# LasseWolter/laughter-detection-icsi

Measured on AMD Instinct MI355X. Metric: 1 s@16 kHz segments/sec (featurize+ResNet fwd/bwd), higher is better.
Workload: dtype f32 (64->64 and 32->32 convolutions: f16x2 split operands with per-tile power-of-two scales, f32 accumulate; error vs float64 within 1.5x of the exact-f32 kernels'); 1 GPU; BASELINE configs[2]: end-to-end featurize (HIP fbank 44 mel) + ResNetBigger resnet_base fwd/bwd + clip + Adam, random labels, dropout 0.5; global_batch=512, parallelism=dp1, overlap_wgrad=False, overlap_wgrad_small=True, bf16x3_convs=True, f16x2_convs=True, relu_bits=True, virtual_a1=True

## Files before the change

include/lad_hip.h:

```cpp
#ifndef LAD_HIP_H
#define LAD_HIP_H

#include <stdint.h>

#ifdef __cplusplus
extern "C" {
#endif

#define LAD_VERSION 100

enum lad_status {
    LAD_OK = 0,
    LAD_ERR_INVALID = -1,
    LAD_ERR_HIP = -2,
    LAD_ERR_NOMEM = -3,
    LAD_NOT_COVERED = 1
};

int lad_version(void);
const char *lad_last_error(void);

enum lad_pad_mode {
    LAD_PAD_KALDI_MIRROR = 0,
    LAD_PAD_CENTER_REFLECT = 1,
// ... 53 lines not shown

int64_t lad_act_rows(int64_t batch, int32_t H, int32_t W);

int64_t lad_conv_packed_weight_floats(int32_t cout, int32_t cin, int32_t taps, int32_t mode);
int lad_conv_pack_weights(const float *w, int32_t cout, int32_t cin, int32_t taps, int32_t mode, float *wt,
                          void *stream);
int lad_conv_pack_weights_multi(const void *descs, int32_t n_desc, void *stream);
int64_t lad_conv_num_tiles(int64_t batch, int32_t H, int32_t W);
int lad_conv_fwd(const float *in, const float *wt, const float *bias, const float *addend, float *out,
                 float *stat_partials, int64_t batch, int32_t H, int32_t W, int32_t cin, int32_t cout, int32_t taps,
                 void *stream);
int lad_conv_s2_fwd(const float *in, const float *wt, const float *bias, float *out, float *stat_partials,
                    int64_t batch, int32_t H, int32_t W, int32_t cin, int32_t cout, int32_t taps, void *stream);
int lad_bn_fold(const float *gamma, const float *beta, const float *running_mean, const float *running_var,
                const float *conv_bias, int32_t channels, float *scale, float *shift, void *stream);
int lad_conv_fwd_eval(const float *in, const float *wt, const float *scale, const float *shift, const float *addend,
                      float *out, int64_t batch, int32_t H, int32_t W, int32_t cin, int32_t cout, int32_t taps,
                      int32_t relu, void *stream);
int lad_conv_s2_fwd_eval(const float *in, const float *wt, const float *scale, const float *shift, float *out,
                         int64_t batch, int32_t H, int32_t W, int32_t cin, int32_t cout, int32_t taps, int32_t relu,
                         void *stream);
int lad_upsample2(const float *src, float *up, int64_t batch, int32_t H, int32_t W, int32_t channels, void *stream);
int lad_conv_s2_dgrad(const float *dout, const float *wt, float *dx, int64_t batch, int32_t H, int32_t W, int32_t cin,
                      int32_t cout, int32_t taps, int32_t accumulate, void *stream);
int64_t lad_conv_s2_wgrad_workspace_floats(int32_t cin, int32_t cout, int32_t taps);
int lad_conv_s2_wgrad(const float *in, const float *dout, float *workspace, float *dw, float *dbias, int64_t batch, int32_t H,
                      int32_t W, int32_t cin, int32_t cout, int32_t taps, void *stream);
int64_t lad_conv_s2_wgrad_fused_workspace_floats(int32_t cin, int32_t cout);
int lad_conv_s2_wgrad_fused(const float *in, const float *dout, const float *dout_sc, float *workspace, float *dw,
                            float *dbias, float *dw_sc, int64_t batch, int32_t H, int32_t W, int32_t cin, int32_t cout,
                            void *stream);
int lad_conv_s2_fwd_fused(const float *in, const float *wt, const float *bias, const float *wt_sc, float *out,
                          float *stat_partials, float *out_sc, float *stat_partials_sc, int64_t batch, int32_t H, int32_t W,
                          int32_t cin, int32_t cout, void *stream);
int lad_conv_s2_dgrad_fused(const float *dout, const float *wt, const float *dout_sc, const float *wt_sc, float *dx,
                            int64_t batch, int32_t H, int32_t W, int32_t cin, int32_t cout, void *stream);
int64_t lad_conv_s2b3_packed_weight_bytes(void);
int lad_conv_s2b3_pack_weights(const float *w, const float *w_sc, void *wt, void *stream);
int lad_conv_s2b3_fwd(const float *in, const void *wt, const float *bias, float *out, float *stat_partials, float *out_sc,
                      float *stat_partials_sc, int64_t batch, int32_t H, int32_t W, void *stream);
int64_t lad_conv_s2b3_dgrad_packed_weight_bytes(void);
int lad_conv_s2b3_dgrad_pack_weights(const float *w, const float *w_sc, void *wt, void *stream);
int lad_conv_s2b3_pack_weights_pair(const float *w, const float *w_sc, void *wt_fwd, void *wt_dgrad, void *stream);
int64_t lad_conv_s2b3_dgrad_partials(int64_t batch, int32_t H, int32_t W);
int lad_conv_s2b3_dgrad(const float *dout, const float *dout_sc, const void *wt, float *dx, float *stat_partials, const float *bn_x,
                        const uint64_t *bn_bits, const float *bn_coef, int64_t batch, int32_t H, int32_t W, void *stream);
int64_t lad_conv_s2_dgrad_partials(int64_t batch, int32_t H, int32_t W);
int lad_conv_s2_dgrad_fused_bnstat(const float *dout, const float *wt, const float *dout_sc, const float *wt_sc, float *dx,
                                   float *stat_partials, const float *bn_x, const uint64_t *bn_bits, const float *bn_coef,
                                   int64_t batch, int32_t H, int32_t W, int32_t cin, int32_t cout, void *stream);
int64_t lad_conv_wgrad_workspace_floats(int32_t cin, int32_t cout, int32_t taps);
int lad_conv_wgrad(const float *in, const float *dout, float *workspace, float *dw, float *dbias, int64_t batch,
                   int32_t H, int32_t W, int32_t cin, int32_t cout, int32_t taps, void *stream);

int64_t lad_conv_b3_packed_weight_bytes(void);
int lad_conv_b3_pack_weights(const float *w, int32_t mode, void *wt, void *stream);
int lad_conv_b3_fwd_f32(const float *in, const void *wt, const float *bias, const float *addend, float *out,
                        float *partials, int64_t batch, int32_t H, int32_t W, void *stream);
int lad_conv_b3_fwd_f32_gated(const float *in, const void *wt, const float *bias, const float *addend,
                              const uint64_t *addend_bits, float *out, float *partials, int64_t batch, int32_t H,
                              int32_t W, void *stream);
int lad_conv_b3_dgrad_bnstat(const float *in, const void *wt, const float *addend, const uint64_t *addend_bits,
                             float *out, float *stat_partials, const float *bn_x, const uint64_t *bn_bits,
                             const float *bn_coef, int64_t batch, int32_t H, int32_t W, void *stream);
int64_t lad_conv_b3c_packed_weight_bytes(int32_t channels);
int lad_conv_b3c_pack_weights(const float *w, int32_t mode, void *wt, int32_t channels, void *stream);
int lad_conv_b3c_fwd_f32(const float *in, const void *wt, const float *bias, const float *addend, float *out,
                         float *partials, int64_t batch, int32_t H, int32_t W, int32_t channels, void *stream);
int lad_conv_b3c_dgrad_bnstat(const float *in, const void *wt, const float *addend, float *out, float *stat_partials,
                              const float *bn_x, const float *bn_coef, int64_t batch, int32_t H, int32_t W,
                              int32_t channels, void *stream);
int lad_conv_b3c_fwd_f32_bnrelu(const float *in, const float *in_coef, const void *wt, const float *bias, float *out,
                                float *partials, int64_t batch, int32_t H, int32_t W, int32_t channels, void *stream);
int64_t lad_conv_h2_packed_weight_bytes(int32_t channels);
int lad_conv_h2_pack_weights_multi(const void *table, int32_t n, int32_t channels, void *stream);
int lad_conv_wgrad_h2(const float *in, const float *in_coef, const float *dout, float *workspace, float *dw, float *dbias,
                      int64_t batch, int32_t H, int32_t W, int32_t channels, void *stream);
int lad_conv_wgrad_h2_bnbwd(const float *in, const float *in_coef, const float *dy, const float *bn_x, const uint64_t *bn_bits,
                            const float *bn_coef, const float *bcoef, float *dc, float *workspace, float *dw, float *dbias,
                            int64_t batch, int32_t H, int32_t W, int32_t channels, void *stream);
int lad_conv_h2(const float *in, const float *in_coef, const void *wt, const float *bias, const float *addend,
                const uint64_t *addend_bits, float *out, float *partials, const float *bn_x, const uint64_t *bn_bits,
                const float *bn_coef, int64_t batch, int32_t H, int32_t W, int32_t channels, void *stream);
int64_t lad_conv_wgrad_b3c_workspace_floats(int32_t channels);
int lad_conv_wgrad_b3c(const float *in, const float *in_coef, const float *dout, float *workspace, float *dw, float *dbias,
                       int64_t batch, int32_t H, int32_t W, int32_t channels, void *stream);
int lad_conv_b3_fwd_f32_bnrelu(const float *in, const float *in_coef, const void *wt, const float *bias, float *out,
                               float *partials, int64_t batch, int32_t H, int32_t W, void *stream);
int lad_conv_wgrad_b3_bnrelu(const float *in, const float *in_coef, const float *dout, float *workspace, float *dw,
                             float *dbias, int64_t batch, int32_t H, int32_t W, void *stream);
int lad_wgrad_defer_begin(void);
int lad_wgrad_defer_flush(void *stream);
int lad_conv_wgrad_b3(const float *in, const float *dout, float *workspace, float *dw, float *dbias, int64_t batch,
                      int32_t H, int32_t W, void *stream);

int lad_stem_fwd(const float *feat, const float *weight, float *out, float *stat_partials, int64_t batch, int32_t H,
                 int32_t W, int32_t cout, void *stream);
int lad_stem_fwd_eval(const float *feat, const float *weight, const float *scale, const float *shift, float *out,
                      int64_t batch, int32_t H, int32_t W, int32_t cout, int64_t frame_stride, int64_t frames_avail,
                      void *stream);
int64_t lad_stem_moments_workspace_doubles(void);
int64_t lad_stem_moments_doubles(void);
int lad_stem_bn_stats(const float *feat, const float *weight, const float *gamma, const float *beta, float *running_mean,
                      float *running_var, float momentum, float *coef, double *moments, double *workspace, int64_t batch, int32_t H,
                      int32_t W, int32_t cout, void *stream);
int64_t lad_stem_bwd_onepass_workspace_floats(void);
int lad_stem_bwd_onepass(const float *feat, const float *weight, const float *dy, const float *coef, const float *gamma,
                         const double *moments, float *workspace, float *dw, float *dgamma, float *dbeta, int64_t batch, int32_t H,
                         int32_t W, int32_t cout, void *stream);
int64_t lad_stem_wgrad_workspace_floats(void);
int lad_stem_wgrad(const float *feat, const float *dout, float *workspace, float *dw, int64_t batch, int32_t H,
                   int32_t W, int32_t cout, void *stream);
int lad_stem_wgrad_bn(const float *feat, const float *dy, const float *x, const float *weight, const float *coef,
                      const float *bcoef, float *workspace, float *dw, int64_t batch, int32_t H, int32_t W, int32_t cout,
                      void *stream);
int64_t lad_stem_bn_bwd_groups(int64_t batch, int32_t H, int32_t W);
int lad_stem_bn_bwd_sums(const float *feat, const float *weight, const float *dy, const float *coef, float *partials,
                         int64_t batch, int32_t H, int32_t W, int32_t cout, void *stream);

int lad_bn_finalize(float *stat_partials, int64_t n_tiles, int32_t channels, int64_t count, const float *gamma,
                    const float *beta, float *running_mean, float *running_var, float momentum, float *coef,
                    void *stream);
int lad_bn_finalize_pair(float *stat_partials_a, float *stat_partials_b, int64_t n_tiles, int32_t channels, int64_t count,
                         const float *gamma_a, const float *beta_a, float *running_mean_a, float *running_var_a, float *coef_a,
                         const float *gamma_b, const float *beta_b, float *running_mean_b, float *running_var_b, float *coef_b,
                         float momentum, void *stream);
int lad_bn_act(const float *x, const float *coef, const float *res, const float *res_coef, float *y, int64_t batch,
               int32_t H, int32_t W, int32_t channels, int32_t relu, void *stream);
int64_t lad_bn_bwd_workspace_floats(int32_t channels);
int lad_bn_bwd(const float *dy, const float *y, const float *x, const float *coef, const float *gamma,
               const float *xs, const float *scoef, const float *sgamma, float *dx, float *aux, float *dgamma,
               float *dbeta, float *dsgamma, float *dsbeta, float *workspace, float *bcoef, float *pre_partials,
               int64_t pre_tiles, int64_t batch, int32_t H, int32_t W, int32_t channels, int32_t relu, int32_t mode,
               void *stream);
int lad_bn_act_bits(const float *x, const float *coef, const float *res, const float *res_coef, float *y,
                    uint64_t *y_bits, int64_t batch, int32_t H, int32_t W, int32_t channels, void *stream);
int lad_bn_bwd_bits(const float *dy, const uint64_t *y_bits, const float *x, const float *coef, const float *gamma,
                    float *dx, float *dgamma, float *dbeta, float *workspace, float *bcoef, float *pre_partials,
                    int64_t pre_tiles, int64_t batch, int32_t H, int32_t W, int32_t channels, void *stream);
int lad_conv_fwd_bnstat(const float *in, const float *wt, const float *addend, float *out, float *stat_partials,
                        const float *bn_x, const float *bn_y, const float *bn_coef, int64_t batch, int32_t H, int32_t W,
                        int32_t cin, int32_t cout, int32_t taps, void *stream);

int lad_pool_fwd(const float *x, float *pooled, int64_t batch, int32_t H, int32_t W, int32_t channels, void *stream);
int lad_pool_bwd(const float *dpooled, float *dx, int64_t batch, int32_t H, int32_t W, int32_t channels, void *stream);
int64_t lad_head_workspace_floats(int64_t batch, int32_t F);
int lad_head_fwd_train(const float *const *params, const float *pooled, int64_t batch, int32_t F, const float *drop1,
                       const float *drop2, const int32_t *labels, float momentum, float *h, float *stats,
                       float *probs, float *metrics, void *stream);
int lad_head_fwd_train_rng(const float *const *params, const float *pooled, int64_t batch, int32_t F, float *drop1, float *drop2, float keep,
                           uint64_t seed, int64_t *rng_counter, int64_t *nbt, int32_t n_nbt, const int32_t *labels, float momentum,
                           float *h, float *stats, float *probs, float *metrics, void *stream);
int lad_head_fwd_eval(const float *const *params, const float *pooled, int64_t batch, int32_t F, float *probs,
                      void *stream);
int lad_bce_metrics(const float *probs, const int32_t *labels, int64_t n, float *metrics, void *stream);
int lad_head_bwd(const float *const *params, float *const *grads, const float *pooled, const float *h,
                 const float *stats, const float *probs, const float *dprobs, int64_t batch, int32_t F,
                 const float *drop1, const float *drop2, const int32_t *labels, float *workspace, float *dpooled,
                 void *stream);

int64_t lad_f16_packed_weight_halfs(int32_t cout, int32_t cin, int32_t taps);
int lad_f16_pack_weights(const float *w, int32_t cout, int32_t cin, int32_t taps, void *wt, void *stream);
int lad_f16_stem_fwd(const float *feat, const float *weight, const float *scale, const float *shift, void *out,
                     int64_t batch, int32_t H, int32_t W, int32_t cout, int64_t frame_stride, int64_t frames_avail,
                     void *stream);
int lad_f16_conv_fwd(const void *in, const void *wt, const float *scale, const float *shift, const void *addend, void *out,
// ... 162 lines not shown
```

laughter-detection-icsi_amd/_hip.py:

```python
import ctypes
import os

import numpy as np
import torch

_HERE = os.path.dirname(os.path.abspath(__file__))
LIB_PATH = os.environ.get("LAD_HIP_LIB") or os.path.join(_HERE, "liblad_hip.so")

c_void_p = ctypes.c_void_p
c_int = ctypes.c_int
c_i64 = ctypes.c_int64
c_float = ctypes.c_float
c_double = ctypes.c_double
c_i32 = ctypes.c_int32
c_float_p = ctypes.POINTER(ctypes.c_float)


class LadHipError(RuntimeError):
    pass


class FbankCfg(ctypes.Structure):
    _fields_ = [("n_fft", ctypes.c_int32), ("frame_len", ctypes.c_int32), ("hop", ctypes.c_int32),
                ("n_mels", ctypes.c_int32), ("n_mfcc", ctypes.c_int32), ("pad_mode", ctypes.c_int32),
                ("log_mode", ctypes.c_int32), ("remove_dc", ctypes.c_int32), ("preemph", ctypes.c_float),
                ("log_floor", ctypes.c_float)]


class AugmentParams(ctypes.Structure):
    _fields_ = [("seed", ctypes.c_uint64), ("epoch", ctypes.c_uint32), ("p", ctypes.c_float), ("mix_p", ctypes.c_float),
                ("snr_lo", ctypes.c_float), ("snr_hi", ctypes.c_float), ("gain_lo", ctypes.c_float), ("gain_hi", ctypes.c_float),
                ("W", ctypes.c_int32), ("n_time", ctypes.c_int32), ("Wt", ctypes.c_int32), ("n_freq", ctypes.c_int32),
                ("Wf", ctypes.c_int32)]


SIGNATURES = {
    "lad_version": (c_int, []),
    "lad_last_error": (ctypes.c_char_p, []),
    "lad_fbank_plan_create": (c_int, [ctypes.POINTER(FbankCfg), c_void_p, c_void_p, c_void_p,
                                      ctypes.POINTER(c_void_p)]),
    "lad_fbank_plan_destroy": (c_int, [c_void_p]),
    "lad_fbank_plan_set_kernel": (c_int, [c_void_p, c_int]),
    "lad_fbank_plan_has_fast_kernel": (c_int, [c_void_p]),
    "lad_fbank_num_frames": (c_i64, [c_void_p, c_i64]),
    "lad_fbank_forward": (c_int, [c_void_p, c_void_p, c_i64, c_i64, c_void_p, c_void_p]),
    "lad_fbank_forward_long": (c_int, [c_void_p, c_void_p, c_i64, c_void_p, c_void_p]),
    "lad_gather_segments": (c_int, [c_void_p] * 5 + [c_i64, c_i32, c_i32, c_float, c_void_p, c_void_p]),
    "lad_gather_segments_aug": (c_int, [c_void_p] * 5 + [c_i64, c_i32, c_i32, c_float, ctypes.POINTER(AugmentParams), c_void_p, c_i32, c_i64,
                                        c_void_p, c_void_p]),
    "lad_assemble_windows": (c_int, [c_void_p, c_void_p, c_void_p, c_i64, c_i32, c_i32, c_i32, c_i32, c_void_p]),
    "lad_act_rows": (c_i64, [c_i64, c_i32, c_i32]),
    "lad_conv_packed_weight_floats": (c_i64, [c_i32, c_i32, c_i32, c_i32]),
    "lad_conv_pack_weights": (c_int, [c_void_p, c_i32, c_i32, c_i32, c_i32, c_void_p, c_void_p]),
    "lad_conv_pack_weights_multi": (c_int, [c_void_p, c_i32, c_void_p]),
    "lad_conv_num_tiles": (c_i64, [c_i64, c_i32, c_i32]),
    "lad_conv_fwd": (c_int, [c_void_p] * 6 + [c_i64, c_i32, c_i32, c_i32, c_i32, c_i32, c_void_p]),
    "lad_conv_b3_packed_weight_bytes": (c_i64, []),
    "lad_conv_b3_pack_weights": (c_int, [c_void_p, c_i32, c_void_p, c_void_p]),
    "lad_conv_b3_fwd_f32": (c_int, [c_void_p] * 6 + [c_i64, c_i32, c_i32, c_void_p]),
    "lad_conv_b3c_packed_weight_bytes": (c_i64, [c_i32]),
    "lad_conv_b3c_pack_weights": (c_int, [c_void_p, c_i32, c_void_p, c_i32, c_void_p]),
    "lad_conv_b3c_fwd_f32": (c_int, [c_void_p] * 6 + [c_i64, c_i32, c_i32, c_i32, c_void_p]),
    "lad_conv_b3c_fwd_f32_bnrelu": (c_int, [c_void_p] * 6 + [c_i64, c_i32, c_i32, c_i32, c_void_p]),
    "lad_conv_b3c_dgrad_bnstat": (c_int, [c_void_p] * 7 + [c_i64, c_i32, c_i32, c_i32, c_void_p]),
    "lad_conv_h2_packed_weight_bytes": (c_i64, [c_i32]),
    "lad_conv_h2_pack_weights_multi": (c_int, [c_void_p, c_i32, c_i32, c_void_p]),
    "lad_conv_wgrad_h2": (c_int, [c_void_p] * 6 + [c_i64, c_i32, c_i32, c_i32, c_void_p]),
    "lad_conv_h2": (c_int, [c_void_p] * 11 + [c_i64, c_i32, c_i32, c_i32, c_void_p]),
    "lad_conv_wgrad_h2_bnbwd": (c_int, [c_void_p] * 11 + [c_i64, c_i32, c_i32, c_i32, c_void_p]),
    "lad_conv_wgrad_b3c_workspace_floats": (c_i64, [c_i32]),
    "lad_conv_wgrad_b3c": (c_int, [c_void_p] * 6 + [c_i64, c_i32, c_i32, c_i32, c_void_p]),
    "lad_conv_b3_fwd_f32_gated": (c_int, [c_void_p] * 7 + [c_i64, c_i32, c_i32, c_void_p]),
    "lad_conv_b3_fwd_f32_bnrelu": (c_int, [c_void_p] * 6 + [c_i64, c_i32, c_i32, c_void_p]),
    "lad_conv_wgrad_b3_bnrelu": (c_int, [c_void_p] * 6 + [c_i64, c_i32, c_i32, c_void_p]),
    "lad_wgrad_defer_begin": (c_int, []),
    "lad_wgrad_defer_flush": (c_int, [c_void_p]),
    "lad_conv_b3_dgrad_bnstat": (c_int, [c_void_p] * 9 + [c_i64, c_i32, c_i32, c_void_p]),
    "lad_conv_wgrad_b3": (c_int, [c_void_p] * 5 + [c_i64, c_i32, c_i32, c_void_p]),
    "lad_conv_s2_fwd": (c_int, [c_void_p] * 5 + [c_i64, c_i32, c_i32, c_i32, c_i32, c_i32, c_void_p]),
    "lad_bn_fold": (c_int, [c_void_p] * 5 + [c_i32, c_void_p, c_void_p, c_void_p]),
    "lad_conv_fwd_eval": (c_int, [c_void_p] * 6 + [c_i64, c_i32, c_i32, c_i32, c_i32, c_i32, c_i32, c_void_p]),
    "lad_conv_s2_fwd_eval": (c_int, [c_void_p] * 5 + [c_i64, c_i32, c_i32, c_i32, c_i32, c_i32, c_i32, c_void_p]),
    "lad_upsample2": (c_int, [c_void_p, c_void_p, c_i64, c_i32, c_i32, c_i32, c_void_p]),
    "lad_conv_s2_dgrad": (c_int, [c_void_p] * 3 + [c_i64, c_i32, c_i32, c_i32, c_i32, c_i32, c_i32, c_void_p]),
    "lad_conv_s2_wgrad_workspace_floats": (c_i64, [c_i32, c_i32, c_i32]),
    "lad_conv_s2_fwd_fused": (c_int, [c_void_p] * 8 + [c_i64, c_i32, c_i32, c_i32, c_i32, c_void_p]),
    "lad_conv_s2_dgrad_partials": (c_i64, [c_i64, c_i32, c_i32]),
    "lad_conv_s2b3_packed_weight_bytes": (c_i64, []),
    "lad_conv_s2b3_pack_weights": (c_int, [c_void_p, c_void_p, c_void_p, c_void_p]),
    "lad_conv_s2b3_fwd": (c_int, [c_void_p] * 7 + [c_i64, c_i32, c_i32, c_void_p]),
    "lad_conv_s2b3_dgrad_packed_weight_bytes": (c_i64, []),
    "lad_conv_s2b3_dgrad_pack_weights": (c_int, [c_void_p, c_void_p, c_void_p, c_void_p]),
    "lad_conv_s2b3_pack_weights_pair": (c_int, [c_void_p] * 5),
    "lad_conv_s2b3_dgrad_partials": (c_i64, [c_i64, c_i32, c_i32]),
    "lad_conv_s2b3_dgrad": (c_int, [c_void_p] * 8 + [c_i64, c_i32, c_i32, c_void_p]),
    "lad_conv_s2_dgrad_fused_bnstat": (c_int, [c_void_p] * 9 + [c_i64, c_i32, c_i32, c_i32, c_i32, c_void_p]),
    "lad_conv_s2_dgrad_fused": (c_int, [c_void_p] * 5 + [c_i64, c_i32, c_i32, c_i32, c_i32, c_void_p]),
    "lad_conv_s2_wgrad_fused_workspace_floats": (c_i64, [c_i32, c_i32]),
    "lad_conv_s2_wgrad_fused": (c_int, [c_void_p] * 7 + [c_i64, c_i32, c_i32, c_i32, c_i32, c_void_p]),
    "lad_conv_s2_wgrad": (c_int, [c_void_p] * 5 + [c_i64, c_i32, c_i32, c_i32, c_i32, c_i32, c_void_p]),
    "lad_conv_wgrad_workspace_floats": (c_i64, [c_i32, c_i32, c_i32]),
    "lad_conv_wgrad": (c_int, [c_void_p] * 5 + [c_i64, c_i32, c_i32, c_i32, c_i32, c_i32, c_void_p]),
    "lad_stem_fwd": (c_int, [c_void_p] * 4 + [c_i64, c_i32, c_i32, c_i32, c_void_p]),
    "lad_stem_fwd_eval": (c_int, [c_void_p] * 5 + [c_i64, c_i32, c_i32, c_i32, c_i64, c_i64, c_void_p]),
    "lad_stem_wgrad_workspace_floats": (c_i64, []),
    "lad_stem_wgrad": (c_int, [c_void_p] * 4 + [c_i64, c_i32, c_i32, c_i32, c_void_p]),
    "lad_stem_wgrad_bn": (c_int, [c_void_p] * 8 + [c_i64, c_i32, c_i32, c_i32, c_void_p]),
    "lad_stem_bn_bwd_groups": (c_i64, [c_i64, c_i32, c_i32]),
    "lad_stem_bn_bwd_sums": (c_int, [c_void_p] * 5 + [c_i64, c_i32, c_i32, c_i32, c_void_p]),
    "lad_bn_finalize": (c_int, [c_void_p, c_i64, c_i32, c_i64, c_void_p, c_void_p, c_void_p, c_void_p, c_float,
                                c_void_p, c_void_p]),
    "lad_stem_moments_workspace_doubles": (c_i64, []),
    "lad_stem_moments_doubles": (c_i64, []),
    "lad_stem_bn_stats": (c_int, [c_void_p] * 6 + [c_float] + [c_void_p] * 3 + [c_i64, c_i32, c_i32, c_i32, c_void_p]),
    "lad_stem_bwd_onepass_workspace_floats": (c_i64, []),
    "lad_stem_bwd_onepass": (c_int, [c_void_p] * 10 + [c_i64, c_i32, c_i32, c_i32, c_void_p]),
    "lad_bn_finalize_pair": (c_int, [c_void_p, c_void_p, c_i64, c_i32, c_i64] + [c_void_p] * 10 + [c_float, c_void_p]),
    "lad_bn_act": (c_int, [c_void_p] * 5 + [c_i64, c_i32, c_i32, c_i32, c_i32, c_void_p]),
    "lad_bn_bwd_workspace_floats": (c_i64, [c_i32]),
    "lad_bn_act_bits": (c_int, [c_void_p] * 6 + [c_i64, c_i32, c_i32, c_i32, c_void_p]),
    "lad_bn_bwd_bits": (c_int, [c_void_p] * 11 + [c_i64, c_i64, c_i32, c_i32, c_i32, c_void_p]),
    "lad_bn_bwd": (c_int, [c_void_p] * 17 + [c_i64, c_i64, c_i32, c_i32, c_i32, c_i32, c_i32, c_void_p]),
    "lad_conv_fwd_bnstat": (c_int, [c_void_p] * 8 + [c_i64, c_i32, c_i32, c_i32, c_i32, c_i32, c_void_p]),
    "lad_pool_fwd": (c_int, [c_void_p, c_void_p, c_i64, c_i32, c_i32, c_i32, c_void_p]),
    "lad_pool_bwd": (c_int, [c_void_p, c_void_p, c_i64, c_i32, c_i32, c_i32, c_void_p]),
    "lad_head_workspace_floats": (c_i64, [c_i64, c_i32]),
    "lad_head_fwd_train": (c_int, [c_void_p, c_void_p, c_i64, c_i32, c_void_p, c_void_p, c_void_p, c_float,
                                   c_void_p, c_void_p, c_void_p, c_void_p, c_void_p]),
    "lad_head_fwd_train_rng": (c_int, [c_void_p, c_void_p, c_i64, c_i32, c_void_p, c_void_p, c_float, ctypes.c_uint64, c_void_p, c_void_p, c_i32,
                                       c_void_p, c_float, c_void_p, c_void_p, c_void_p, c_void_p, c_void_p]),
    "lad_head_fwd_eval": (c_int, [c_void_p, c_void_p, c_i64, c_i32, c_void_p, c_void_p]),
    "lad_bce_metrics": (c_int, [c_void_p, c_void_p, c_i64, c_void_p, c_void_p]),
    "lad_head_bwd": (c_int, [c_void_p] * 7 + [c_i64, c_i32] + [c_void_p] * 6),
    "lad_f16_packed_weight_halfs": (c_i64, [c_i32, c_i32, c_i32]),
    "lad_f16_pack_weights": (c_int, [c_void_p, c_i32, c_i32, c_i32, c_void_p, c_void_p]),
    "lad_f16_stem_fwd": (c_int, [c_void_p] * 5 + [c_i64, c_i32, c_i32, c_i32, c_i64, c_i64, c_void_p]),
    "lad_f16_conv_fwd": (c_int, [c_void_p] * 6 + [c_i64, c_i32, c_i32, c_i32, c_i32, c_i32, c_i32, c_void_p]),
    "lad_f16_block_fwd": (c_int, [c_void_p] * 8 + [c_i64, c_i32, c_i32, c_i32, c_void_p]),
    "lad_f16_conv_s2_fwd_sc": (c_int, [c_void_p] * 9 + [c_i64, c_i32, c_i32, c_i32, c_i32, c_i32, c_void_p]),
    "lad_f16_conv_s2_fwd_mapped_sc": (c_int, [c_void_p] * 9 + [c_i64, c_i32, c_i32, c_i32, c_i32, c_i64, c_i64, c_i32, c_i64, c_i64, c_i32,
                                              c_i32, c_i32, c_i32, c_void_p]),
    "lad_f16_conv_s2_fwd": (c_int, [c_void_p] * 5 + [c_i64, c_i32, c_i32, c_i32, c_i32, c_i32, c_i32, c_void_p]),
    "lad_f16_conv_s2_fwd_windows": (c_int, [c_void_p] * 5 + [c_i64, c_i32, c_i32, c_i32, c_i32, c_i32, c_i32, c_i32, c_void_p]),
    "lad_f16_conv_s2_fwd_mapped": (c_int, [c_void_p] * 5 + [c_i64, c_i32, c_i32, c_i32, c_i32, c_i64, c_i64, c_i32, c_i64, c_i64, c_i32,
                                                          c_i32, c_i32, c_i32, c_i32, c_void_p]),
    "lad_f16_block_fwd_stem_rows": (c_int, [c_void_p, c_i64, c_i64, c_void_p, c_i64] + [c_void_p] * 10 + [c_i64, c_i32, c_i32, c_void_p]),
    "lad_f16_conv_s2_strips_fwd": (c_int, [c_void_p] * 9 + [c_i64, c_i32, c_i32, c_i32, c_i32, c_i64, c_i64, c_i64, c_i32, c_void_p]),
    "lad_f16_tail_fwd": (c_int, [c_void_p, c_i64, c_i32, c_i32, c_i32, c_i32, c_i64, c_i64, c_i32, c_i64, c_i64, c_void_p, c_void_p, c_i32,
                                 c_void_p, c_void_p]),
    "lad_f16_pool_fwd": (c_int, [c_void_p, c_void_p, c_i64, c_i32, c_i32, c_i32, c_void_p]),
    "lad_grad_sumsq_partials": (c_i32, []),
# ... 157 lines not shown
```

laughter-detection-icsi_amd/csrc/conv_h2.hip:

```cpp
#include "lad_common.h"
#include "lad_device.h"
#include "lad_b3_tile.h"
#include "lad_bn_math.h"
#include "lad_h2.h"

#include <algorithm>
#include <cstdlib>

namespace {
using namespace lad;
using namespace lad::b3t;

constexpr int KC = 32;
constexpr int ROWB = 128;
constexpr int FPIECES = KC * 4 / 16;

template <int C>
struct H2 {
    static constexpr int NSTAGE = C / KC;
    static constexpr int NCT = C / 16;
    static constexpr int PLANE_B = NCT * 1024;
    static constexpr int TAP_BYTES = 2 * PLANE_B;
    static constexpr int IMG_BYTES = TAPS * NSTAGE * TAP_BYTES;
    static constexpr int TAIL_BYTES = 16;
};

struct PackRec {
    const float *w;
    unsigned char *wt;
    int mode;
    int channels;
};
constexpr int PACK_SPLIT = 16;
template <int C>
__device__ __forceinline__ void pack_h2_image(const PackRec &rec, int part) {
    using K = H2<C>;
    __shared__ float smax[K::NSTAGE][16];
    __shared__ int kexp[K::NSTAGE];
    const int tid = threadIdx.x, lane = tid & 63, wave = tid >> 6;
    float m[K::NSTAGE];
#pragma unroll
    for (int s = 0; s < K::NSTAGE; ++s) m[s] = 0.f;
    static_assert((C * TAPS) % 4 == 0, "float4 groups stay inside one (co, ci range)");
    for (int idx4 = tid; idx4 < C * C * TAPS / 4; idx4 += 1024) {
        const float4 v = reinterpret_cast<const float4 *>(rec.w)[idx4];
        const float a[4] = {fabsf(v.x), fabsf(v.y), fabsf(v.z), fabsf(v.w)};
#pragma unroll
        for (int j = 0; j < 4; ++j) {
            const int idx = idx4 * 4 + j;
            const int co = idx / (C * TAPS), ci = (idx / TAPS) % C;
            const int k = rec.mode == 0 ? ci : co;
#pragma unroll
            for (int s = 0; s < K::NSTAGE; ++s) m[s] = (k / KC == s) ? fmaxf(m[s], a[j]) : m[s];
        }
    }
#pragma unroll
    for (int s = 0; s < K::NSTAGE; ++s) {
        const float v = wave_max64_dpp(m[s]);
        if (lane == 0) smax[s][wave] = v;
    }
    __syncthreads();
    if (tid < K::NSTAGE) {
        float v = 0.f;
        for (int w = 0; w < 16; ++w) v = fmaxf(v, smax[tid][w]);
        kexp[tid] = scale_exp(v);
        if (part == 0) reinterpret_cast<int *>(rec.wt + K::IMG_BYTES)[tid] = kexp[tid];
    }
    __syncthreads();
    unsigned short *out = reinterpret_cast<unsigned short *>(rec.wt);
    constexpr int SHARE = K::IMG_BYTES / 2 / PACK_SPLIT;
    for (int idx = part * SHARE + tid; idx < (part + 1) * SHARE; idx += 1024) {
        int t = idx;
        const int e = t & 7; t >>= 3;
        const int n = t & 15; t >>= 4;
        const int kq = t & 3; t >>= 2;
        const int ct = t % K::NCT; t /= K::NCT;
        const int plane = t & 1; t >>= 1;
        const int stage = t % K::NSTAGE;
        const int tap = t / K::NSTAGE;
        const int k = stage * KC + kq * 8 + e;
        const int nn = ct * 16 + n;
        const int co = rec.mode == 0 ? nn : k, ci = rec.mode == 0 ? k : nn;
        const int src_tap = rec.mode == 0 ? tap : TAPS - 1 - tap;
        const float v = rec.w[((int64_t)co * C + ci) * TAPS + src_tap] * pow2f(kexp[stage]);
        const _Float16 h1 = (_Float16)v;
        const _Float16 h2 = (_Float16)(v - (float)h1);
        out[idx] = __builtin_bit_cast(unsigned short, plane == 0 ? h1 : h2);
    }
}
template <int C>
__global__ __launch_bounds__(1024) void pack_h2_kernel(const PackRec *__restrict__ recs) {
    const PackRec rec = recs[blockIdx.x / PACK_SPLIT];
    const int part = blockIdx.x % PACK_SPLIT;
    if (C == 64 || (C == 0 && rec.channels == 64)) pack_h2_image<64>(rec, part);
    else pack_h2_image<32>(rec, part);
}

#ifdef LAD_STAMP
__device__ unsigned long long lad_dbg_h2[16 * 16384];
#define LAD_H2_STAMP(k) \
    if (threadIdx.x == 0 && blockIdx.x < 16384) lad_dbg_h2[blockIdx.x * 16 + (k)] = __builtin_amdgcn_s_memtime();
#else
#define LAD_H2_STAMP(k)
#endif

constexpr int NSLOT = 3;
constexpr int H2_EPI_ANY = -1;
constexpr int h2_epi(bool bias, int addend, bool partials, bool from_bits) {
    return (bias ? 1 : 0) | (addend << 1) | (partials ? 8 : 0) | (from_bits ? 16 : 0);
}
template <int C, int RB, bool STAT, bool INBN, int EPI>
__global__ __launch_bounds__(THREADS, RB == 1 ? 3 : 2) void conv_h2_kernel(const float *__restrict__ in, const unsigned char *__restrict__ wt,
                                                             const float *__restrict__ bias, const float *addend,
                                                             const unsigned long long *__restrict__ abits, float *out,
                                                             float *__restrict__ partials, Geom g, B3Stat bst,
                                                             const float *__restrict__ in_coef) {
    using K = H2<C>;
    constexpr int NSTAGE = K::NSTAGE, NCT = K::NCT, PLANE_B = K::PLANE_B, TAP_BYTES = K::TAP_BYTES;
    constexpr int TMW = TM * RB, NRT = 2 * RB;
    constexpr int NPRE = ((TMW + 2 * 47) * FPIECES + THREADS - 1) / THREADS;
    constexpr int CPS = TAPS;
    constexpr int KP = (CPS - NSLOT) < CPS / 2 ? (CPS - NSLOT) : CPS / 2;
    static_assert(CPS % NSLOT == 0 && NPRE <= 32, "every stage starts in ring slot 0; staging geometry");
    extern __shared__ __attribute__((aligned(128))) unsigned char smem_b[];
    const int tid = threadIdx.x, lane = tid & 63, wave = __builtin_amdgcn_readfirstlane(tid >> 6);
    const int halo = g.Wp + 1;
    const int nrows = TMW + 2 * halo;
    const int main_bytes = max(NSLOT * TAP_BYTES + nrows * ROWB, TM * (C + 4) * 4);
    unsigned char *b_s = smem_b;
    unsigned char *a_s = b_s + NSLOT * TAP_BYTES;
    unsigned char *mask_s = smem_b + main_bytes;
    float *smax = reinterpret_cast<float *>(mask_s + TMW);
    const unsigned per_x = (gridDim.x + 7u) / 8u;
    const unsigned tile_id = (blockIdx.x % 8u) * per_x + blockIdx.x / 8u;
    const int64_t q0 = (int64_t)tile_id * TMW;
    if (q0 >= g.rows) return;

    LAD_H2_STAMP(0)
    constexpr int NW_TAP = TAP_BYTES / (THREADS * 16);
    static_assert(TAP_BYTES % (THREADS * 16) == 0 && NW_TAP >= 1, "the DMA count per tap must not depend on the wave");
    auto issue_tap = [&](int tap, int stage, int slot) {
        const unsigned char *src = wt + (int64_t)(tap * NSTAGE + stage) * TAP_BYTES;
        unsigned char *dst = b_s + slot * TAP_BYTES;
#pragma unroll
        for (int r = 0; r < NW_TAP; ++r)
            dma16(src + (r * THREADS + tid) * 16, lds_addr(dst + (r * THREADS + wave * 64) * 16));
    };
    const int *wexp = reinterpret_cast<const int *>(wt + K::IMG_BYTES);

    const int64_t start = q0 - halo;
    const int64_t first = start < 0 ? 0 : start;
    const int row_lo = (int)(first - start);
    const int64_t span_rows = min(g.rows - first, (int64_t)(nrows - row_lo));
    auto voff = [&](int u) {
        const int idx = u * THREADS + tid;
        return idx < nrows * FPIECES ? ((idx >> 3) - row_lo) * (C * 4) + (idx & 7) * 16 : -1;
    };
    auto stage_rsrc = [&](int stage) {
        return make_rsrc(reinterpret_cast<const unsigned char *>(in) + first * (C * 4) + stage * (KC * 4), span_rows * (C * 4) - stage * (KC * 4));
    };
    unsigned keep_bits = 0;
    u32x4 pre[NPRE];
    auto activate = [&](int stage) {
        float m = 0.f;
        f32x4 sc = {0.f, 0.f, 0.f, 0.f}, sh = sc;
        if (INBN) {
            sc = *reinterpret_cast<const f32x4 *>(in_coef + stage * KC + (tid & 7) * 4);
            sh = *reinterpret_cast<const f32x4 *>(in_coef + C + stage * KC + (tid & 7) * 4);
        }
#pragma unroll
        for (int u = 0; u < NPRE; ++u) {
            if (INBN) pre[u] = bn_relu_piece(pre[u], sc, sh, (keep_bits >> u) & 1u);
            const float4 f = as_f4(pre[u]);
            m = fmaxf(fmaxf(m, fmaxf(fabsf(f.x), fabsf(f.y))), fmaxf(fabsf(f.z), fabsf(f.w)));
        }
        m = wave_max64_dpp(m);
        if (lane == 0) smax[wave] = m;
    };
    auto tile_exp = [&]() { return scale_exp(fmaxf(fmaxf(smax[0], smax[1]), fmaxf(smax[2], smax[3]))); };
    auto put_all = [&](float scl) {
#pragma unroll
        for (int u = 0; u < NPRE; ++u) {
            const int idx = u * THREADS + tid;
            if (idx < nrows * FPIECES) {
                const int row = idx >> 3, piece = idx & 7;
                const float4 f = as_f4(pre[u]);
                unsigned a1, a2, b1, b2;
                split2_pair(f.x * scl, f.y * scl, a1, a2);
                split2_pair(f.z * scl, f.w * scl, b1, b2);
                const unsigned off = (unsigned)row * ROWB + ((((piece >> 1) ^ (row & 6)) << 4) | ((piece & 1) << 3));
                *reinterpret_cast<u32x2 *>(a_s + off) = u32x2{a1, b1};
                *reinterpret_cast<u32x2 *>(a_s + (off ^ 64u)) = u32x2{a2, b2};
            }
        }
    };

    {
        const __amdgpu_buffer_rsrc_t in_r = stage_rsrc(0);
#pragma unroll
        for (int u = 0; u < NPRE; ++u) pre[u] = buf_load16(in_r, voff(u));
    }
#pragma unroll
    for (int k = 0; k < NSLOT - 1; ++k) issue_tap(k, 0, k);
    for (int j = tid; j < TMW; j += THREADS) mask_s[j] = interior_row32((uint32_t)q0 + (uint32_t)j, g) ? 1 : 0;
    if (INBN) {
#pragma unroll
        for (int u = 0; u < NPRE; ++u)
            keep_bits |= (interior_row32((uint32_t)(start + ((u * THREADS + tid) >> 3)), g) ? 1u : 0u) << u;
    }
    LAD_H2_STAMP(1)
    activate(0);
    __syncthreads();
    int ktot = tile_exp() + wexp[0];
    put_all(pow2f(ktot - wexp[0]));
    LAD_H2_STAMP(2)

    const int m = lane & 15, kq = lane >> 4;
    const int rl = wave * 32 + m + halo - 1;
    const unsigned char *b_lane = b_s + kq * 256 + m * 16;

    f32x4 acc[NRT][NCT];
#pragma unroll
    for (int r = 0; r < NRT; ++r)
#pragma unroll
        for (int c = 0; c < NCT; ++c) acc[r][c] = f32x4{0.f, 0.f, 0.f, 0.f};

#pragma unroll
    for (int stage = 0; stage < NSTAGE; ++stage) {
        const bool last = stage + 1 == NSTAGE;
#pragma unroll
        for (int tap = 0; tap < TAPS; ++tap) {
            const int kc = tap;
            const int slot = kc % NSLOT;
            {
                constexpr int YOUNGER = NSLOT - 2;
                if (!last) {
                    if (kc > KP && kc <= KP + NSLOT - 1) wait_dma_fixed<YOUNGER, NPRE, NW_TAP>();
                    else wait_dma_fixed<YOUNGER, 0, NW_TAP>();
                } else {
                    if (CPS - 1 - kc >= YOUNGER) wait_dma_fixed<YOUNGER, 0, NW_TAP>();
                    else wait_dma_fixed<0, 0, NW_TAP>();
                }
                __syncthreads();
                const int kn = kc + NSLOT - 1;
                if (kn < CPS) issue_tap(kn, stage, kn % NSLOT);
                else if (!last) issue_tap(kn - CPS, stage + 1, kn % NSLOT);
                if (kc == KP && !last) {
                    const __amdgpu_buffer_rsrc_t in_r = stage_rsrc(stage + 1);
#pragma unroll
                    for (int u = 0; u < NPRE; ++u) pre[u] = buf_load16(in_r, voff(u));
                }
            }
            const int rt = rl + (tap / 3 - 1) * g.Wp + (tap % 3);
            const unsigned a1o = (unsigned)rt * ROWB + ((unsigned)(kq ^ (rt & 6)) << 4);
            const unsigned a2o = a1o ^ 64u;
            const int boff = slot * TAP_BYTES;
            f16x8 a1[NRT], a2[NRT];
#pragma unroll
            for (int r = 0; r < NRT; ++r) {
                const int roff = ((r >> 1) * TM + (r & 1) * 16) * ROWB;
                a1[r] = *reinterpret_cast<const f16x8 *>(a_s + a1o + roff);
                a2[r] = *reinterpret_cast<const f16x8 *>(a_s + a2o + roff);
            }
#pragma unroll
            for (int c = 0; c < NCT; ++c) {
                const f16x8 b1 = *reinterpret_cast<const f16x8 *>(b_lane + boff + c * 1024);
                const f16x8 b2 = *reinterpret_cast<const f16x8 *>(b_lane + boff + PLANE_B + c * 1024);
#pragma unroll
                for (int r = 0; r < NRT; ++r) acc[r][c] = __builtin_amdgcn_mfma_f32_16x16x32_f16(a1[r], b2, acc[r][c], 0, 0, 0);
#pragma unroll
                for (int r = 0; r < NRT; ++r) acc[r][c] = __builtin_amdgcn_mfma_f32_16x16x32_f16(a2[r], b1, acc[r][c], 0, 0, 0);
#pragma unroll
                for (int r = 0; r < NRT; ++r) acc[r][c] = __builtin_amdgcn_mfma_f32_16x16x32_f16(a1[r], b1, acc[r][c], 0, 0, 0);
            }
        }
#ifdef LAD_STAMP
        if (threadIdx.x == 0 && blockIdx.x < 16384) lad_dbg_h2[blockIdx.x * 16 + 3 + 2 * stage] = __builtin_amdgcn_s_memtime();
#endif
        if (!last) {
            activate(stage + 1);
            __syncthreads();
            const int kw = wexp[stage + 1];
            const int kn = min(tile_exp() + kw, ktot + 8);
            const int d = kn - ktot;
            if (d != 0) {
#pragma unroll
                for (int r = 0; r < NRT; ++r)
#pragma unroll
                    for (int c = 0; c < NCT; ++c)
#pragma unroll
                        for (int j = 0; j < 4; ++j) acc[r][c][j] = __builtin_ldexpf(acc[r][c][j], d);
            }
            ktot = kn;
            const int ka = kn - kw;
            put_all(ka >= -126 ? pow2f(ka) : 0.f);
        }
#ifdef LAD_STAMP
        if (threadIdx.x == 0 && blockIdx.x < 16384) lad_dbg_h2[blockIdx.x * 16 + 4 + 2 * stage] = __builtin_amdgcn_s_memtime();
#endif
    }
    __syncthreads();
    LAD_H2_STAMP(11)
#pragma unroll
    for (int rb = 0; rb < RB; ++rb) {
        const int64_t qs = q0 + rb * TM;
        if (rb > 0) {
            if (qs >= g.rows) break;
            __syncthreads();
        }
        auto store_acc = [&](float *my) {
#pragma unroll
            for (int rr = 0; rr < 2; ++rr)
#pragma unroll
                for (int c = 0; c < NCT; ++c)
#pragma unroll
                    for (int j = 0; j < 4; ++j)
                        my[(rr * 16 + (lane >> 4) * 4 + j) * (C + 4) + c * 16 + m] = __builtin_ldexpf(acc[rb * 2 + rr][c][j], -ktot);
        };
        if constexpr (EPI == H2_EPI_ANY)
            b3_epilogue<C, STAT>(store_acc, bias, addend, abits, out, partials, mask_s + rb * TM, reinterpret_cast<float *>(smem_b), qs, g.rows, bst);
        else
            h2_epilogue<C, STAT, (EPI & 1) != 0, (EPI >> 1) & 3, (EPI & 8) != 0, (EPI & 16) != 0>(
                store_acc, bias, addend, abits, out, partials, mask_s + rb * TM, reinterpret_cast<float *>(smem_b), qs, g.rows, bst);
    }
    LAD_H2_STAMP(12)
}

template <int C, int RB>
size_t h2_lds_bytes(const Geom &g) {
    using K = H2<C>;
    const int nrows = TM * RB + 2 * (g.Wp + 1);
    const size_t main_bytes = std::max<size_t>(NSLOT * K::TAP_BYTES + (size_t)nrows * ROWB, (size_t)TM * (C + 4) * 4);
    return main_bytes + TM * RB + 16;
}

int h2_two_rounds() {
    static int n = 0;
    if (n == 0) {
        int dev = 0;
        hipDeviceProp_t prop;
        n = (hipGetDevice(&dev) == hipSuccess && hipGetDeviceProperties(&prop, dev) == hipSuccess && prop.multiProcessorCount > 0)
                ? 4 * prop.multiProcessorCount : 1024;
    }
    return n;
}

struct H2Args {
    const float *in, *in_coef;
    const unsigned char *wt;
    const float *bias, *addend;
    const unsigned long long *abits;
    float *out, *partials;
    B3Stat bst;
    Geom g;
    hipStream_t stream;
};

template <int C, int RB, bool STAT, bool INBN, int EPI>
int launch_h2_form(const H2Args &a) {
    static lad::DeviceOnce attr_set;
    if (!attr_set) {
        LAD_HIP_CHECK(hipFuncSetAttribute((const void *)conv_h2_kernel<C, RB, STAT, INBN, EPI>, hipFuncAttributeMaxDynamicSharedMemorySize, 96 * 1024));
        attr_set = true;
    }
    const int64_t tiles = ceil_div(a.g.rows, TM * RB);
    hipLaunchKernelGGL((conv_h2_kernel<C, RB, STAT, INBN, EPI>), dim3((unsigned)(ceil_div(tiles, 8) * 8)), dim3(THREADS), (h2_lds_bytes<C, RB>(a.g)),
                       a.stream, a.in, a.wt, a.bias, a.addend, a.abits, a.out, a.partials, a.g, a.bst, a.in_coef);
    return check_launch("conv_h2_kernel");
}

template <int C, int RB, bool STAT, bool INBN>
int launch_h2_rb(const H2Args &a) {
    const int form = h2_epi(a.bias != nullptr, a.addend == nullptr ? H2_ADD_NONE : a.abits == nullptr ? H2_ADD_PLAIN : H2_ADD_GATED,
                            a.partials != nullptr, STAT && a.bst.bits != nullptr);
#define LAD_H2_FORM(...)                                                                                                           \
    if (form == h2_epi(__VA_ARGS__)) return launch_h2_form<C, RB, STAT, INBN, h2_epi(__VA_ARGS__)>(a);
    if constexpr (STAT) {
        LAD_H2_FORM(false, H2_ADD_NONE, true, false)
        LAD_H2_FORM(false, H2_ADD_GATED, true, true)
    } else {
        LAD_H2_FORM(true, H2_ADD_NONE, true, false)
        LAD_H2_FORM(true, H2_ADD_PLAIN, true, false)
        if constexpr (!INBN) {
            LAD_H2_FORM(false, H2_ADD_NONE, false, false)
            LAD_H2_FORM(false, H2_ADD_PLAIN, false, false)
            LAD_H2_FORM(false, H2_ADD_GATED, false, false)
        }
    }
#undef LAD_H2_FORM
    return launch_h2_form<C, RB, STAT, INBN, H2_EPI_ANY>(a);
}

template <int C, bool STAT, bool INBN>
int launch_h2(const float *in, const float *in_coef, const void *wt, const float *bias, const float *addend, const uint64_t *abits,
              float *out, float *partials, const B3Stat &bst, int64_t batch, int32_t H, int32_t W, void *stream, const char *who) {
    const Geom g = make_geom(batch, H, W);
    LAD_REQUIRE(g.rows < ((int64_t)1 << 31) && g.img < (1 << 20), "%s: more than 2^31 rows, or an image of more than 2^20 positions", who);
    LAD_REQUIRE(W <= 46, "%s: image too wide for the tile (W = %d)", who, W);
    const H2Args a{in, in_coef, (const unsigned char *)wt, bias, addend, (const unsigned long long *)abits, out, partials, bst, g, (hipStream_t)stream};
    if (ceil_div(g.rows, TM * 2) < h2_two_rounds()) return launch_h2_rb<C, 1, STAT, INBN>(a);
    return launch_h2_rb<C, 2, STAT, INBN>(a);
}
}

extern "C" int64_t lad_conv_h2_packed_weight_bytes(int32_t channels) {
    if (channels == 64) return H2<64>::IMG_BYTES + H2<64>::TAIL_BYTES;
    if (channels == 32) return H2<32>::IMG_BYTES + H2<32>::TAIL_BYTES;
    return -1;
}

extern "C" int lad_conv_h2_pack_weights_multi(const void *table, int32_t n, int32_t channels, void *stream) {
    using namespace lad;
    LAD_REQUIRE(table && n >= 1, "lad_conv_h2_pack_weights_multi: empty table");
    static_assert(sizeof(PackRec) == 24, "record layout");
    if (channels == 64) hipLaunchKernelGGL(pack_h2_kernel<64>, dim3(n * PACK_SPLIT), dim3(1024), 0, (hipStream_t)stream, (const PackRec *)table);
    else if (channels == 32) hipLaunchKernelGGL(pack_h2_kernel<32>, dim3(n * PACK_SPLIT), dim3(1024), 0, (hipStream_t)stream, (const PackRec *)table);
    else if (channels == 0) hipLaunchKernelGGL(pack_h2_kernel<0>, dim3(n * PACK_SPLIT), dim3(1024), 0, (hipStream_t)stream, (const PackRec *)table);
    else return fail(LAD_ERR_INVALID, "lad_conv_h2_pack_weights_multi: 64 or 32 channels, or 0 = per record (got %d)", channels);
    return check_launch("pack_h2_kernel");
}

extern "C" int lad_conv_h2(const float *in, const float *in_coef, const void *wt, const float *bias, const float *addend,
                           const uint64_t *addend_bits, float *out, float *partials, const float *bn_x, const uint64_t *bn_bits,
                           const float *bn_coef, int64_t batch, int32_t H, int32_t W, int32_t channels, void *stream) {
    using namespace lad;
    const char *who = "lad_conv_h2";
    LAD_REQUIRE(batch >= 1 && H >= 1 && W >= 1, "%s: bad geometry", who);
    LAD_REQUIRE(in && wt && out, "%s: null buffer", who);
    LAD_REQUIRE(addend_bits == nullptr || addend != nullptr, "%s: sign bits without an addend", who);
    LAD_REQUIRE((const void *)in != (const void *)out, "%s: the convolution cannot run in place", who);
    const bool stat = bn_x != nullptr;
    LAD_REQUIRE(!stat || (partials && bn_coef), "%s: the BatchNorm sums need partials and bn_coef", who);
    LAD_REQUIRE(stat || bn_bits == nullptr, "%s: bn_bits without bn_x", who);
    LAD_REQUIRE(!(stat && in_coef), "%s: an input BatchNorm and the backward sums are not combined", who);
    LAD_REQUIRE(channels == 64 || (addend_bits == nullptr && bn_bits == nullptr), "%s: sign bits are kept for 64-channel activations only", who);
    const B3Stat bst{bn_x, (const unsigned long long *)bn_bits, bn_coef};
    if (channels == 64) {
        if (stat) return launch_h2<64, true, false>(in, nullptr, wt, bias, addend, addend_bits, out, partials, bst, batch, H, W, stream, who);
        if (in_coef) return launch_h2<64, false, true>(in, in_coef, wt, bias, addend, addend_bits, out, partials, bst, batch, H, W, stream, who);
        return launch_h2<64, false, false>(in, nullptr, wt, bias, addend, addend_bits, out, partials, bst, batch, H, W, stream, who);
    }
    if (channels == 32) {
        if (stat) return launch_h2<32, true, false>(in, nullptr, wt, bias, addend, addend_bits, out, partials, bst, batch, H, W, stream, who);
        if (in_coef) return launch_h2<32, false, true>(in, in_coef, wt, bias, addend, addend_bits, out, partials, bst, batch, H, W, stream, who);
        return launch_h2<32, false, false>(in, nullptr, wt, bias, addend, addend_bits, out, partials, bst, batch, H, W, stream, who);
    }
    return fail(LAD_ERR_INVALID, "%s: 64 or 32 channels (got %d)", who, channels);
}

#ifdef LAD_STAMP
extern "C" int lad_debug_read_h2_stamps(unsigned long long *host_dst, int64_t n) {
    return hipMemcpyFromSymbol(host_dst, HIP_SYMBOL(lad_dbg_h2), n * sizeof(unsigned long long)) == hipSuccess ? 0 : -2;
}
#endif
```

laughter-detection-icsi_amd/csrc/lad_b3_tile.h:

```cpp
#pragma once
#include "lad_common.h"
#include "lad_device.h"

namespace lad {
namespace b3t {

constexpr int TAPS = 9;
constexpr int TM = 128;
constexpr int THREADS = 256;

struct B3Stat {
    const float *x;
    const unsigned long long *bits;
    const float *coef;
};

struct B3Scatter {
    const int *rowoff;
    int64_t base_row;
    int64_t span_rows;
    int64_t part_tile;
};

template <int C, bool STAT, bool SCATTER = false, class StoreAcc, class MaskT>
__device__ __forceinline__ void b3_epilogue(StoreAcc store_acc, const float *__restrict__ bias, const float *addend,
                                            const unsigned long long *__restrict__ abits, float *out, float *__restrict__ partials,
                                            const MaskT *mask_tile, float *out_s, int64_t q0, int64_t rows, const B3Stat &bst,
                                            const B3Scatter &sct = B3Scatter{nullptr, 0, 0, 0}) {
    constexpr int LDO = C + 4, LPR = C / 4, RPI = 64 / LPR, ITER = 32 / RPI, STEP = RPI * C * 4;
    const int tid = (int)threadIdx.x, lane = tid & 63, wave = tid >> 6;
    float *my = out_s + wave * 32 * LDO;
    store_acc(my);
    const int c4 = lane % LPR, rsub = lane / LPR;
    const int64_t row0 = SCATTER ? sct.base_row : q0;
    const int64_t tile_rows = SCATTER ? sct.span_rows : rows - q0;
    const int64_t tile_bytes = tile_rows * (C * 4);
    const int voff = ((wave * 32 + rsub) * C + c4 * 4) * 4;
    const int woff = (wave * 32 + rsub) * 8;
    int ro[SCATTER ? ITER : 1];
    if (SCATTER) {
#pragma unroll
        for (int it = 0; it < ITER; ++it) ro[it] = sct.rowoff[wave * 32 + it * RPI + rsub];
    }
    auto off16 = [&](int it) { return SCATTER ? (ro[SCATTER ? it : 0] < 0 ? -1 : ro[SCATTER ? it : 0] * (C * 4) + c4 * 16) : voff + it * STEP; };
    auto off8 = [&](int it) { return SCATTER ? (ro[SCATTER ? it : 0] < 0 ? -1 : ro[SCATTER ? it : 0] * 8) : woff + it * RPI * 8; };
    const __amdgpu_buffer_rsrc_t out_r = make_rsrc(out + row0 * C, tile_bytes);
    f32x4 bv = {0.f, 0.f, 0.f, 0.f};
    if (bias != nullptr) bv = *reinterpret_cast<const f32x4 *>(bias + c4 * 4);
    f32x4 s1 = {0.f, 0.f, 0.f, 0.f}, s2 = s1;
    f32x4 fsc = s1, fsh = s1, mu = s1, is = s1, mul = s1, isl = s1;
    if (STAT) {
        fsc = *reinterpret_cast<const f32x4 *>(bst.coef + 0 * C + c4 * 4);
        fsh = *reinterpret_cast<const f32x4 *>(bst.coef + 1 * C + c4 * 4);
        mu = *reinterpret_cast<const f32x4 *>(bst.coef + 2 * C + c4 * 4);
        is = *reinterpret_cast<const f32x4 *>(bst.coef + 3 * C + c4 * 4);
        mul = *reinterpret_cast<const f32x4 *>(bst.coef + 4 * C + c4 * 4);
        isl = *reinterpret_cast<const f32x4 *>(bst.coef + 5 * C + c4 * 4);
    }
    const bool from_bits = STAT && bst.bits != nullptr;
    auto gate = [&](u32x4 v, u32x2 w) {
        const unsigned lo = w.x >> c4, hi = w.y >> c4;
        v.x = (lo & 1u) ? v.x : 0u;
        v.y = (lo & 0x10000u) ? v.y : 0u;
        v.z = (hi & 1u) ? v.z : 0u;
        v.w = (hi & 0x10000u) ? v.w : 0u;
        return v;
    };
    constexpr int NI = STAT ? ITER / 2 : ITER;
#pragma unroll
    for (int i0 = 0; i0 < ITER; i0 += NI) {
        u32x4 adv[NI], bx[STAT ? NI : 1];
        u32x2 wv[NI], bw[STAT ? NI : 1];
        if (addend != nullptr) {
            const __amdgpu_buffer_rsrc_t add_r = make_rsrc(addend + row0 * C, tile_bytes);
#pragma unroll
            for (int u = 0; u < NI; ++u) adv[u] = buf_load16(add_r, off16(i0 + u));
            if (abits != nullptr) {
                const __amdgpu_buffer_rsrc_t bits_r = make_rsrc(abits + row0, tile_rows * 8);
#pragma unroll
                for (int u = 0; u < NI; ++u) wv[u] = buf_load8(bits_r, off8(i0 + u));
            }
        }
        if (STAT) {
            const __amdgpu_buffer_rsrc_t x_r = make_rsrc(bst.x + row0 * C, tile_bytes);
#pragma unroll
// ... 86 lines not shown
        const unsigned lo = w.x >> c4, hi = w.y >> c4;
        v.x = (lo & 1u) ? v.x : 0u;
        v.y = (lo & 0x10000u) ? v.y : 0u;
        v.z = (hi & 1u) ? v.z : 0u;
        v.w = (hi & 0x10000u) ? v.w : 0u;
        return v;
    };
    constexpr int NI = (STAT || ADDEND == H2_ADD_GATED) ? ITER / 2 : ITER;
#pragma unroll
    for (int i0 = 0; i0 < ITER; i0 += NI) {
        u32x4 adv[ADDEND != H2_ADD_NONE ? NI : 1], bx[STAT ? NI : 1];
        u32x2 wv[ADDEND == H2_ADD_GATED ? NI : 1], bw[FROM_BITS ? NI : 1];
        if constexpr (ADDEND != H2_ADD_NONE) {
            const __amdgpu_buffer_rsrc_t add_r = make_rsrc(addend + q0 * C, tile_bytes);
#pragma unroll
            for (int u = 0; u < NI; ++u) adv[u] = buf_load16(add_r, voff + (i0 + u) * STEP);
            if constexpr (ADDEND == H2_ADD_GATED) {
                const __amdgpu_buffer_rsrc_t bits_r = make_rsrc(abits + q0, tile_rows * 8);
#pragma unroll
                for (int u = 0; u < NI; ++u) wv[u] = buf_load8(bits_r, woff + (i0 + u) * RPI * 8);
            }
        }
        if constexpr (STAT) {
            const __amdgpu_buffer_rsrc_t x_r = make_rsrc(bst.x + q0 * C, tile_bytes);
#pragma unroll
            for (int u = 0; u < NI; ++u) bx[u] = buf_load16(x_r, voff + (i0 + u) * STEP);
            if constexpr (FROM_BITS) {
                const __amdgpu_buffer_rsrc_t w_r = make_rsrc(bst.bits + q0, tile_rows * 8);
#pragma unroll
                for (int u = 0; u < NI; ++u) bw[u] = buf_load8(w_r, woff + (i0 + u) * RPI * 8);
            }
        }
#pragma unroll
        for (int u = 0; u < NI; ++u) {
            const int it = i0 + u;
            const int row = it * RPI + rsub;
            const float keep = (float)mask_tile[wave * 32 + row];
            f32x4 t = *reinterpret_cast<const f32x4 *>(my + row * LDO + c4 * 4);
            t += bv;
            if constexpr (ADDEND == H2_ADD_GATED) t += __builtin_bit_cast(f32x4, gate(adv[u], wv[u]));
            else if constexpr (ADDEND == H2_ADD_PLAIN) t += __builtin_bit_cast(f32x4, adv[u]);
            t *= keep;
            buf_store16(__builtin_bit_cast(u32x4, t), out_r, voff + it * STEP);
            if constexpr (!STAT) {
                if constexpr (HAS_PARTIALS) {
                    s1 += t;
                    s2 = __builtin_elementwise_fma(t, t, s2);
                }
            } else {
                const f32x4 xv = __builtin_bit_cast(f32x4, bx[u]);
                f32x4 d;
                if constexpr (FROM_BITS) {
                    d = __builtin_bit_cast(f32x4, gate(__builtin_bit_cast(u32x4, t), bw[u]));
                } else {
                    const f32x4 yv = __builtin_elementwise_fma(xv, fsc, fsh);
                    d.x = yv.x > 0.f ? t.x : 0.f;
                    d.y = yv.y > 0.f ? t.y : 0.f;
                    d.z = yv.z > 0.f ? t.z : 0.f;
                    d.w = yv.w > 0.f ? t.w : 0.f;
                }
                const f32x4 tx = (xv - mu) - mul;
                const f32x4 xh = __builtin_elementwise_fma(tx, is, tx * isl);
                s1 += d;
                s2 = __builtin_elementwise_fma(d, xh, s2);
            }
        }
    }
    if constexpr (HAS_PARTIALS) {
        *reinterpret_cast<f32x4 *>(my + (rsub * 2 + 0) * C + c4 * 4) = s1;
        *reinterpret_cast<f32x4 *>(my + (rsub * 2 + 1) * C + c4 * 4) = s2;
        __syncthreads();
        if (tid < 2 * C) {
            const int k = tid / C, co = tid - k * C;
            float s = 0.0f;
#pragma unroll
            for (int w = 0; w < 4; ++w)
#pragma unroll
                for (int rs = 0; rs < RPI; ++rs) s += out_s[w * 32 * LDO + (rs * 2 + k) * C + co];
            partials[(q0 / TM * 2 + k) * C + co] = s;
        }
    }
}

template <int TAP_BYTES>
__device__ __forceinline__ int dma_per_tap(int wave) {
    int n = 0;
#pragma unroll
    for (int r = 0; r * THREADS * 16 < TAP_BYTES; ++r) n += ((r * THREADS + wave * 64) * 16 < TAP_BYTES) ? 1 : 0;
    return n;
}

template <int TAPS_YOUNGER, int EXTRA>
__device__ __forceinline__ void wait_dma(int nw_tap) {
    static_assert(2 * TAPS_YOUNGER + EXTRA <= 63, "vmcnt is a 6-bit field");
    if (nw_tap == 2) asm volatile("s_waitcnt vmcnt(%0)" ::"n"(2 * TAPS_YOUNGER + EXTRA) : "memory");
    else if (nw_tap == 1) asm volatile("s_waitcnt vmcnt(%0)" ::"n"(TAPS_YOUNGER + EXTRA) : "memory");
    else asm volatile("s_waitcnt vmcnt(%0)" ::"n"(EXTRA) : "memory");
}
template <int TAPS_YOUNGER, int EXTRA, int NW_TAP>
__device__ __forceinline__ void wait_dma_fixed() {
    static_assert(NW_TAP * TAPS_YOUNGER + EXTRA <= 63, "vmcnt is a 6-bit field");
    asm volatile("s_waitcnt vmcnt(%0)" ::"n"(NW_TAP * TAPS_YOUNGER + EXTRA) : "memory");
}

}
}
```

laughter-detection-icsi_amd/csrc/lad_common.h:

```cpp
#pragma once
#include <hip/hip_runtime.h>

#include <atomic>
#include <cstdarg>
#include <cstdint>
#include <cstdio>
#include <string>

#include "../../include/lad_hip.h"

namespace lad {

std::string &last_error_ref();
int fail(int code, const char *fmt, ...);

#define LAD_HIP_CHECK(expr)                                                                         \
    do {                                                                                            \
        hipError_t _e = (expr);                                                                     \
        if (_e != hipSuccess)                                                                       \
            return ::lad::fail(LAD_ERR_HIP, "%s failed: %s (%s:%d)", #expr, hipGetErrorString(_e), \
                               __FILE__, __LINE__);                                                 \
    } while (0)

#define LAD_REQUIRE(cond, ...)                                   \
    do {                                                         \
        if (!(cond)) return ::lad::fail(LAD_ERR_INVALID, __VA_ARGS__); \
    } while (0)

inline int check_launch(const char *what) {
    hipError_t e = hipGetLastError();
    if (e != hipSuccess) return fail(LAD_ERR_HIP, "launch of %s failed: %s", what, hipGetErrorString(e));
    return LAD_OK;
}

struct DeviceOnce {
    std::atomic<uint64_t> mask[4] = {};
    static int dev() {
        int d = 0;
        (void)hipGetDevice(&d);
        return d & 255;
    }
    bool operator!() const { const int d = dev(); return !((mask[d >> 6].load(std::memory_order_acquire) >> (d & 63)) & 1); }
    DeviceOnce &operator=(bool) {
        const int d = dev();
        mask[d >> 6].fetch_or(1ull << (d & 63), std::memory_order_release);
        return *this;
    }
};

inline int64_t ceil_div(int64_t a, int64_t b) { return (a + b - 1) / b; }
inline int64_t up256(int64_t bytes) { return (bytes + 255) / 256 * 256; }

struct SlabReduce {
    const float *slabs, *bias_slabs;
    float *dw, *dbias;
    int groups, cin, cout, taps;
};
int reduce_slabs(const SlabReduce &d, hipStream_t st);

unsigned int *launch_ticket();

}
```

laughter-detection-icsi_amd/csrc/lad_device.h:

```cpp
#pragma once
#include <hip/hip_runtime.h>

#include <cstdint>

namespace lad {

typedef float f32x16 __attribute__((ext_vector_type(16)));
typedef float f32x4 __attribute__((ext_vector_type(4)));

struct Geom {
    int64_t rows;
    int64_t body;
    int Hp, Wp;
    int img;
    uint32_t wp_magic;
    double inv_img;
};

__host__ __device__ inline Geom make_geom(int64_t batch, int H, int W) {
    Geom g;
    g.Hp = H + 1;
    g.Wp = W + 1;
    g.img = g.Hp * g.Wp;
    g.body = batch * g.img;
    g.rows = g.body + g.Wp + 1;
    g.wp_magic = (uint32_t)((1ull << 32) / (uint64_t)g.Wp) + 1u;
    g.inv_img = 1.0 / (double)g.img;
    return g;
}

__device__ __forceinline__ bool interior_row(int64_t q, const Geom &g) {
    if (q < 0 || q >= g.body) return false;
    const int rr = (int)(q % g.img);
    const int yp = rr / g.Wp;
    const int xp = rr - yp * g.Wp;
    return (yp >= 1) & (xp >= 1);
}

__device__ __forceinline__ bool interior_row32(uint32_t q, const Geom &g) {
    const uint32_t img = (uint32_t)g.img;
    uint32_t rr = q - (uint32_t)((double)q * g.inv_img) * img;
    rr = rr >= img ? rr - img : rr;
    const uint32_t yp = __umulhi(rr, g.wp_magic);
    const uint32_t xp = rr - yp * (uint32_t)g.Wp;
    return ((int64_t)q < g.body) & (yp >= 1u) & (xp >= 1u);
}

typedef unsigned int u32x4 __attribute__((ext_vector_type(4)));
__device__ __forceinline__ __amdgpu_buffer_rsrc_t make_rsrc(const void *base, int64_t bytes) {
    const uint32_t n = bytes > 0x7fffffffll ? 0x7fffffffu : (bytes < 0 ? 0u : (uint32_t)bytes);
    return __builtin_amdgcn_make_buffer_rsrc(const_cast<void *>(base), 0, n, 0x00020000);
}
__device__ __forceinline__ u32x4 buf_load16(__amdgpu_buffer_rsrc_t r, int byte_off) {
    return __builtin_amdgcn_raw_buffer_load_b128(r, byte_off, 0, 0);
}
__device__ __forceinline__ void buf_store16(u32x4 v, __amdgpu_buffer_rsrc_t r, int byte_off) {
    __builtin_amdgcn_raw_buffer_store_b128(v, r, byte_off, 0, 0);
}
typedef unsigned int u32x2 __attribute__((ext_vector_type(2)));
__device__ __forceinline__ u32x2 buf_load8(__amdgpu_buffer_rsrc_t r, int byte_off) {
    return __builtin_amdgcn_raw_buffer_load_b64(r, byte_off, 0, 0);
}
__device__ __forceinline__ void buf_store8(u32x2 v, __amdgpu_buffer_rsrc_t r, int byte_off) {
    __builtin_amdgcn_raw_buffer_store_b64(v, r, byte_off, 0, 0);
}
__device__ __forceinline__ float4 as_f4(u32x4 v) { return __builtin_bit_cast(float4, v); }
__device__ __forceinline__ u32x4 as_u4(float4 v) { return __builtin_bit_cast(u32x4, v); }

__device__ __forceinline__ f32x16 mfma32(float a, float b, f32x16 c) {
    return __builtin_amdgcn_mfma_f32_32x32x2f32(a, b, c, 0, 0, 0);
}

__device__ __forceinline__ int acc_row(int r, int lane) { return (r & 3) + 8 * (r >> 2) + 4 * (lane >> 5); }

__device__ __forceinline__ float wave_sum64(float v) {
#pragma unroll
    for (int off = 32; off > 0; off >>= 1) v += __shfl_xor(v, off, 64);
    return v;
}

__device__ __forceinline__ double wave_sum64d(double v) {
#pragma unroll
    for (int off = 32; off > 0; off >>= 1) v += __shfl_xor(v, off, 64);
    return v;
}


__device__ __forceinline__ float wave_max64_dpp(float v) {
    int x = __builtin_bit_cast(int, v);
    x = __builtin_bit_cast(int, fmaxf(__builtin_bit_cast(float, x), __builtin_bit_cast(float, __builtin_amdgcn_mov_dpp(x, 0xB1, 0xf, 0xf, true))));
    x = __builtin_bit_cast(int, fmaxf(__builtin_bit_cast(float, x), __builtin_bit_cast(float, __builtin_amdgcn_mov_dpp(x, 0x4E, 0xf, 0xf, true))));
    x = __builtin_bit_cast(int, fmaxf(__builtin_bit_cast(float, x), __builtin_bit_cast(float, __builtin_amdgcn_mov_dpp(x, 0x141, 0xf, 0xf, true))));
    x = __builtin_bit_cast(int, fmaxf(__builtin_bit_cast(float, x), __builtin_bit_cast(float, __builtin_amdgcn_mov_dpp(x, 0x140, 0xf, 0xf, true))));
    const float r0 = __builtin_bit_cast(float, __builtin_amdgcn_readlane(x, 0)), r1 = __builtin_bit_cast(float, __builtin_amdgcn_readlane(x, 16));
    const float r2 = __builtin_bit_cast(float, __builtin_amdgcn_readlane(x, 32)), r3 = __builtin_bit_cast(float, __builtin_amdgcn_readlane(x, 48));
    return fmaxf(fmaxf(r0, r1), fmaxf(r2, r3));
}

typedef _Float16 f16x8 __attribute__((ext_vector_type(8)));
typedef _Float16 f16x4 __attribute__((ext_vector_type(4)));

__device__ __forceinline__ f32x16 mfma32_f16(f16x8 a, f16x8 b, f32x16 c) {
    return __builtin_amdgcn_mfma_f32_32x32x16_f16(a, b, c, 0, 0, 0);
}

__device__ __forceinline__ void dma16(const void *gsrc, unsigned lds_byte_addr) {
    unsigned keep;
    const unsigned dst = __builtin_amdgcn_readfirstlane(lds_byte_addr);
    asm volatile("s_mov_b32 %0, m0\n\ts_mov_b32 m0, %2\n\ts_nop 0\n\tglobal_load_lds_dwordx4 %1, off\n\ts_mov_b32 m0, %0"
                 : "=&s"(keep)
                 : "v"(gsrc), "s"(dst)
                 : "memory");
}
__device__ __forceinline__ void dma16s(const void *uniform_base, unsigned lane_byte_off, unsigned lds_byte_addr) {
    unsigned keep;
    const unsigned dst = __builtin_amdgcn_readfirstlane(lds_byte_addr);
    const unsigned long long b = (unsigned long long)(size_t)uniform_base;
    const unsigned lo = __builtin_amdgcn_readfirstlane((unsigned)b), hi = __builtin_amdgcn_readfirstlane((unsigned)(b >> 32));
    const unsigned long long sb = ((unsigned long long)hi << 32) | lo;
    asm volatile("s_mov_b32 %0, m0\n\ts_mov_b32 m0, %3\n\ts_nop 0\n\tglobal_load_lds_dwordx4 %1, %2\n\ts_mov_b32 m0, %0"
                 : "=&s"(keep)
                 : "v"(lane_byte_off), "s"(sb), "s"(dst)
                 : "memory");
}
__device__ __forceinline__ void dma_wait_all() { asm volatile("s_waitcnt vmcnt(0)" ::: "memory"); }
__device__ __forceinline__ unsigned lds_addr(const void *p) {
    return (unsigned)(size_t)(const __attribute__((address_space(3))) void *)p;
// ... 4 lines not shown
```

laughter-detection-icsi_amd/csrc/lad_stem_taps.h:

```cpp
#pragma once
#include "lad_device.h"

namespace lad {

constexpr int STEM_TM = 128;
constexpr int TAPW = 12;
__device__ __forceinline__ void fill_taps(const float *__restrict__ feat, const Geom &g, int H, int W, int64_t q0,
                                          int64_t frame_stride, int64_t frames_avail, float *tap_s ) {
    const int r = threadIdx.x;
    if (r < STEM_TM) {
        const int64_t q = q0 + r;
        float v[9];
#pragma unroll
        for (int t = 0; t < 9; ++t) v[t] = 0.0f;
        float flag = 0.0f;
        if (q < g.body) {
            const int64_t b = q / g.img;
            const int rr = (int)(q - b * g.img);
            const int yp = rr / g.Wp, xp = rr - yp * g.Wp;
            if (yp >= 1 && xp >= 1) {
                flag = 1.0f;
                const int y = yp - 1, x = xp - 1;
                const int64_t f0 = b * frame_stride;
#pragma unroll
                for (int ky = 0; ky < 3; ++ky)
#pragma unroll
                    for (int kx = 0; kx < 3; ++kx) {
                        const int yy = y + ky - 1, xx = x + kx - 1;
                        const bool ok = yy >= 0 && yy < H && xx >= 0 && xx < W && (f0 + yy) < frames_avail;
                        v[ky * 3 + kx] = ok ? feat[(f0 + yy) * W + xx] : 0.0f;
                    }
            }
        }
        float4 *dst = reinterpret_cast<float4 *>(tap_s + r * TAPW);
        dst[0] = make_float4(v[0], v[1], v[2], v[3]);
        dst[1] = make_float4(v[4], v[5], v[6], v[7]);
        dst[2] = make_float4(v[8], flag, 0.f, 0.f);
    }
}
__device__ __forceinline__ bool read_taps(const float *tap_s, int r, float (&v)[9]) {
    const float4 *src = reinterpret_cast<const float4 *>(tap_s + r * TAPW);
    const float4 a = src[0], b = src[1], c = src[2];
    v[0] = a.x; v[1] = a.y; v[2] = a.z; v[3] = a.w; v[4] = b.x; v[5] = b.y; v[6] = b.z; v[7] = b.w; v[8] = c.x;
    return c.y != 0.0f;
}


}
```

laughter-detection-icsi_amd/csrc/stem.hip:

```cpp
#include "lad_common.h"
#include "lad_device.h"
#include "lad_stem_taps.h"
#include "lad_bn_math.h"

namespace {
using namespace lad;

constexpr int THREADS = 256;
constexpr int TM = lad::STEM_TM;
constexpr int COUT = 64;
constexpr int CQ = COUT / 4;
constexpr int RL = THREADS / CQ;
constexpr int MAX_GROUPS = 1536;

template <bool STORE>
__global__ __launch_bounds__(THREADS) void stem_fwd_kernel(const float *__restrict__ feat, const float *__restrict__ w ,
                                                           float *__restrict__ out, float *__restrict__ partials, Geom g,
                                                           int H, int W) {
    const int tid = threadIdx.x, cq = tid % CQ, rl = tid / CQ;
    float wr[4][9];
#pragma unroll
    for (int c = 0; c < 4; ++c)
#pragma unroll
        for (int t = 0; t < 9; ++t) wr[c][t] = w[(cq * 4 + c) * 9 + t];
// ... 382 lines not shown
        if (running_mean != nullptr) {
            const double unbiased = count > 1.0 ? var * count / (count - 1.0) : var;
            running_mean[c] = (1.0f - momentum) * running_mean[c] + momentum * (float)mean;
            running_var[c] = (1.0f - momentum) * running_var[c] + momentum * (float)unbiased;
        }
    }
}

constexpr int BWD1_COLS = COUT * 9 + 2 * COUT;
__global__ __launch_bounds__(THREADS) void stem_bwd_onepass_kernel(const float *__restrict__ feat, const float *__restrict__ w,
                                                                   const float *__restrict__ dy, const float *__restrict__ coef,
                                                                   const double *__restrict__ mom, float *__restrict__ slabs, Geom g, int H,
                                                                   int W, int64_t n_tiles) {
    const int tid = threadIdx.x, cq = tid % CQ, rl = tid / CQ;
    float acc[4][9];
#pragma unroll
    for (int c = 0; c < 4; ++c)
#pragma unroll
        for (int t = 0; t < 9; ++t) acc[c][t] = 0.f;
    float wr[4][9];
#pragma unroll
    for (int c = 0; c < 4; ++c)
#pragma unroll
        for (int t = 0; t < 9; ++t) wr[c][t] = w[(cq * 4 + c) * 9 + t];
    const float4 fsc = *reinterpret_cast<const float4 *>(coef + cq * 4);
    const float4 fsh = *reinterpret_cast<const float4 *>(coef + COUT + cq * 4);
    const Norm4 nm = load_norm(coef, COUT, cq * 4);
    const float m = (float)mom[MOM_N];
    float4 a0 = make_float4(0.f, 0.f, 0.f, 0.f), a1 = a0;
    __shared__ __attribute__((aligned(16))) float tap_s[TM * TAPW];
    constexpr int NR = TM / RL;
    for (int64_t tile = blockIdx.x; tile < n_tiles; tile += gridDim.x) {
        const int64_t q0 = tile * TM;
        float4 dv[NR];
#pragma unroll
        for (int k = 0; k < NR; ++k) {
            const int64_t q = q0 + rl + k * RL;
            dv[k] = q < g.rows ? *reinterpret_cast<const float4 *>(dy + q * COUT + cq * 4) : make_float4(0.f, 0.f, 0.f, 0.f);
        }
        __syncthreads();
        fill_taps(feat, g, H, W, q0, H, (int64_t)1 << 62, tap_s);
        __syncthreads();
#pragma unroll
        for (int k = 0; k < NR; ++k) {
            const int r = rl + k * RL;
            const int64_t q = q0 + r;
            if (q >= g.rows) break;
            float v[9];
            if (read_taps(tap_s, r, v)) {
                float xa[4] = {0, 0, 0, 0};
#pragma unroll
                for (int t = 0; t < 9; ++t)
#pragma unroll
                    for (int c = 0; c < 4; ++c) xa[c] = fmaf(v[t], wr[c][t], xa[c]);
                const float4 xv = make_float4(xa[0], xa[1], xa[2], xa[3]);
                const float4 d = mask_from_x(dv[k], xv, fsc, fsh);
                const float4 xh = xhat4(xv, nm);
                a0.x += d.x; a0.y += d.y; a0.z += d.z; a0.w += d.w;
                a1.x = fmaf(d.x, xh.x, a1.x); a1.y = fmaf(d.y, xh.y, a1.y); a1.z = fmaf(d.z, xh.z, a1.z); a1.w = fmaf(d.w, xh.w, a1.w);
                const float dd[4] = {d.x, d.y, d.z, d.w};
#pragma unroll
                for (int t = 0; t < 9; ++t) {
                    const float gt = v[t] - m;
#pragma unroll
                    for (int c = 0; c < 4; ++c) acc[c][t] = fmaf(gt, dd[c], acc[c][t]);
                }
            }
        }
    }
    __shared__ float red[RL][BWD1_COLS];
#pragma unroll
    for (int c = 0; c < 4; ++c)
#pragma unroll
        for (int t = 0; t < 9; ++t) red[rl][(cq * 4 + c) * 9 + t] = acc[c][t];
    *reinterpret_cast<float4 *>(&red[rl][COUT * 9 + cq * 4]) = a0;
    *reinterpret_cast<float4 *>(&red[rl][COUT * 10 + cq * 4]) = a1;
    __syncthreads();
    for (int e = tid; e < BWD1_COLS; e += THREADS) {
        float sacc = 0.f;
#pragma unroll
        for (int p = 0; p < RL; ++p) sacc += red[p][e];
        slabs[(int64_t)blockIdx.x * BWD1_COLS + e] = sacc;
    }
}
__global__ __launch_bounds__(64 * CS_PARTS) void stem_bwd_finish_kernel(const float *__restrict__ slabs, float *sums, int groups,
                                                                        const double *__restrict__ mom, const float *__restrict__ w,
                                                                        const float *__restrict__ coef, const float *__restrict__ gamma,
                                                                        float *__restrict__ dw, float *__restrict__ dgamma,
                                                                        float *__restrict__ dbeta, unsigned int *ticket) {
    constexpr int n = BWD1_COLS;
    const int o = threadIdx.x & 63, part = threadIdx.x >> 6;
    const int idx = blockIdx.x * 64 + o;
    __shared__ double red[CS_PARTS][64];
    __shared__ float tot[BWD1_COLS];
    __shared__ int last_s;
    double s = 0.0;
    if (idx < n) {
        const float *src = slabs + idx;
        int wg = part;
        for (; wg + 3 * CS_PARTS < groups; wg += 4 * CS_PARTS) {
            const float a = src[(int64_t)wg * n], b = src[(int64_t)(wg + CS_PARTS) * n], c = src[(int64_t)(wg + 2 * CS_PARTS) * n],
                        d = src[(int64_t)(wg + 3 * CS_PARTS) * n];
            s += (double)a; s += (double)b; s += (double)c; s += (double)d;
        }
        for (; wg < groups; wg += CS_PARTS) s += (double)src[(int64_t)wg * n];
    }
    red[part][o] = s;
    __syncthreads();
    if (part == 0 && idx < n) {
        double t = 0.0;
#pragma unroll
        for (int p = 0; p < CS_PARTS; ++p) t += red[p][o];
        __hip_atomic_store(sums + idx, (float)t, __ATOMIC_RELAXED, __HIP_MEMORY_SCOPE_AGENT);
    }
    asm volatile("s_waitcnt vmcnt(0)" ::: "memory");
    __syncthreads();
    if (threadIdx.x == 0) last_s = __hip_atomic_fetch_add(ticket, 1u, __ATOMIC_RELAXED, __HIP_MEMORY_SCOPE_AGENT) == gridDim.x - 1;
    __syncthreads();
    if (!last_s) return;
    if (threadIdx.x == 0) __hip_atomic_store(ticket, 0u, __ATOMIC_RELAXED, __HIP_MEMORY_SCOPE_AGENT);
    const int e = threadIdx.x;
    if (e < n) tot[e] = __hip_atomic_load(sums + e, __ATOMIC_RELAXED, __HIP_MEMORY_SCOPE_AGENT);
    __syncthreads();
    if (e >= n) return;
    if (e >= COUT * 9) {
        const int c = (e - COUT * 9) & (COUT - 1);
        if (e < COUT * 10) dbeta[c] = tot[e];
        else dgamma[c] = tot[e];
        return;
    }
    const int c = e / 9, t = e - c * 9;
    const double cnt = mom[MOM_N + 1], m = mom[MOM_N];
    const double mean = (double)coef[2 * COUT + c] + (double)coef[4 * COUT + c], invstd = (double)coef[3 * COUT + c] + (double)coef[5 * COUT + c];
    const double k1 = (double)gamma[c] * invstd, k2 = (double)tot[COUT * 9 + c] / cnt, k3 = (double)tot[COUT * 10 + c] / cnt;
    const double g1 = mom[t] - m * cnt;
    double sgx = 0.0;
#pragma unroll
    for (int u = 0; u < 9; ++u) sgx = fma((double)w[c * 9 + u], mom[mom_idx(t, u)] - m * mom[u], sgx);
    const double gx = invstd * (sgx - mean * g1);
    dw[e] = (float)(k1 * ((double)tot[e] - k2 * g1 - k3 * gx));
}

}

extern "C" int lad_stem_fwd(const float *feat, const float *weight, float *out, float *stat_partials, int64_t batch,
                            int32_t H, int32_t W, int32_t cout, void *stream) {
    using namespace lad;
    LAD_REQUIRE(feat && weight && (out || stat_partials), "lad_stem_fwd: null buffer");
    LAD_REQUIRE(cout == COUT, "lad_stem_fwd: cout must be %d", COUT);
    LAD_REQUIRE(batch >= 0 && H >= 1 && W >= 1, "lad_stem_fwd: bad geometry");
    if (batch == 0) return LAD_OK;
    const Geom g = make_geom(batch, H, W);
    if (out != nullptr)
        hipLaunchKernelGGL(stem_fwd_kernel<true>, dim3((unsigned)ceil_div(g.rows, TM)), dim3(THREADS), 0, (hipStream_t)stream, feat,
                           weight, out, stat_partials, g, H, W);
    else
        hipLaunchKernelGGL(stem_fwd_kernel<false>, dim3((unsigned)ceil_div(g.rows, TM)), dim3(THREADS), 0, (hipStream_t)stream, feat,
                           weight, out, stat_partials, g, H, W);
    return check_launch("stem_fwd_kernel");
}

extern "C" int lad_stem_fwd_eval(const float *feat, const float *weight, const float *scale, const float *shift, float *out,
                                 int64_t batch, int32_t H, int32_t W, int32_t cout, int64_t frame_stride, int64_t frames_avail,
                                 void *stream) {
    using namespace lad;
    LAD_REQUIRE(feat && weight && scale && shift && out, "lad_stem_fwd_eval: null buffer");
    LAD_REQUIRE(cout == COUT, "lad_stem_fwd_eval: cout must be %d", COUT);
    LAD_REQUIRE(batch >= 0 && H >= 1 && W >= 1 && frame_stride >= 1 && frames_avail >= 0, "lad_stem_fwd_eval: bad geometry");
    if (batch == 0) return LAD_OK;
    const Geom g = make_geom(batch, H, W);
    hipLaunchKernelGGL(stem_fwd_eval_kernel, dim3((unsigned)ceil_div(g.rows, TM)), dim3(THREADS), 0, (hipStream_t)stream, feat,
                       weight, scale, shift, out, g, H, W, frame_stride, frames_avail);
    return check_launch("stem_fwd_eval_kernel");
}

extern "C" int64_t lad_stem_wgrad_workspace_floats(void) { return (int64_t)MAX_GROUPS * COUT * 9; }

static int stem_wgrad_launch(const float *feat, const float *dout, const float *x, const float *weight, const float *coef,
                             const float *bcoef, float *workspace, float *dw, int64_t batch, int32_t H, int32_t W, void *stream) {
    using namespace lad;
    const Geom g = make_geom(batch, H, W);
    const int64_t n_tiles = ceil_div(g.rows, TM);
    const int groups = (int)std::min<int64_t>(MAX_GROUPS, n_tiles);
    const dim3 grid(groups), block(THREADS);
    hipStream_t st = (hipStream_t)stream;
    if (coef == nullptr)
        hipLaunchKernelGGL(stem_wgrad_kernel<0>, grid, block, 0, st, feat, dout, nullptr, nullptr, nullptr, nullptr, workspace, g, H, W, n_tiles);
    else if (x != nullptr)
        hipLaunchKernelGGL(stem_wgrad_kernel<1>, grid, block, 0, st, feat, dout, x, nullptr, coef, bcoef, workspace, g, H, W, n_tiles);
    else
        hipLaunchKernelGGL(stem_wgrad_kernel<2>, grid, block, 0, st, feat, dout, nullptr, weight, coef, bcoef, workspace, g, H, W, n_tiles);
    int rc = check_launch("stem_wgrad_kernel");
    if (rc) return rc;
    hipLaunchKernelGGL(colsum_kernel, dim3((unsigned)ceil_div(COUT * 9, 64)), dim3(64 * CS_PARTS), 0, st, workspace, dw, groups, COUT * 9);
    return check_launch("colsum_kernel");
}

extern "C" int lad_stem_wgrad(const float *feat, const float *dout, float *workspace, float *dw, int64_t batch, int32_t H,
                              int32_t W, int32_t cout, void *stream) {
    using namespace lad;
    LAD_REQUIRE(feat && dout && workspace && dw, "lad_stem_wgrad: null buffer");
    LAD_REQUIRE(cout == COUT && batch >= 1, "lad_stem_wgrad: bad arguments");
    return stem_wgrad_launch(feat, dout, nullptr, nullptr, nullptr, nullptr, workspace, dw, batch, H, W, stream);
}

extern "C" int lad_stem_wgrad_bn(const float *feat, const float *dy, const float *x, const float *weight, const float *coef,
                                 const float *bcoef, float *workspace, float *dw, int64_t batch, int32_t H, int32_t W, int32_t cout,
                                 void *stream) {
    using namespace lad;
    LAD_REQUIRE(feat && dy && (x || weight) && coef && bcoef && workspace && dw, "lad_stem_wgrad_bn: null buffer");
    LAD_REQUIRE(cout == COUT && batch >= 1, "lad_stem_wgrad_bn: bad arguments");
    return stem_wgrad_launch(feat, dy, x, weight, coef, bcoef, workspace, dw, batch, H, W, stream);
}

extern "C" int64_t lad_stem_bn_bwd_groups(int64_t batch, int32_t H, int32_t W) {
    if (batch < 1 || H < 1 || W < 1) return -1;
    return std::min<int64_t>(MAX_GROUPS, lad::ceil_div(lad::make_geom(batch, H, W).rows, TM));
}

extern "C" int lad_stem_bn_bwd_sums(const float *feat, const float *weight, const float *dy, const float *coef, float *partials,
                                    int64_t batch, int32_t H, int32_t W, int32_t cout, void *stream) {
    using namespace lad;
    LAD_REQUIRE(feat && weight && dy && coef && partials, "lad_stem_bn_bwd_sums: null buffer");
    LAD_REQUIRE(cout == COUT && batch >= 1 && H >= 1 && W >= 1, "lad_stem_bn_bwd_sums: bad arguments");
    const Geom g = make_geom(batch, H, W);
// ... 53 lines not shown
```

laughter-detection-icsi_amd/engine.py:

```python
import ctypes
import math
import struct
from typing import FrozenSet, NamedTuple, Optional, Tuple

import torch

import _hip

_VP = ctypes.c_void_p


PREDICT_CHUNK = {"fp16": 8192, "fp32": 2048}
BASE_WIDTHS = (64, 32, 16, 16)
STREAM_SUPER_MAX = 1 << 20


class _LazyLevels(dict):

    def __init__(self, make):
        super().__init__()
        self._make = make

    def __missing__(self, key):
        value = self[key] = self._make(key)
        return value


def _align4(n):
    return (n + 3) & ~3


def _b3_shape(cin, cout, taps, stride):
    return cin == cout and cin in (64, 32) and taps == 9 and stride == 1


def _s2b3_shape(cin, cout, taps, stride):
    return cin == 64 and cout == 32 and taps == 9 and stride == 2


class _ConvParams:

    def __init__(self, name, cin, cout, taps, stride, base_widths, views, lib, dev):
        self.name, self.cin, self.cout, self.taps = name, cin, cout, taps
        self.w, self.gw = views[name + ".weight"]
        self.b, self.gb = views.get(name + ".bias", (None, None))
        self.shortcut = None

        def image(n, dtype):
            return torch.zeros(int(n), device=dev, dtype=dtype)

        self.wt_f = image(lib.lad_conv_packed_weight_floats(cout, cin, taps, 0), torch.float32)
        self.wt_d = image(lib.lad_conv_packed_weight_floats(cout, cin, taps, 1), torch.float32)
        self.wt_h = image(lib.lad_f16_packed_weight_halfs(cout, cin, taps), torch.float16)
        if _b3_shape(cin, cout, taps, stride) and base_widths:
            self.wt3_f, self.wt3_d = (image(lib.lad_conv_b3c_packed_weight_bytes(cin), torch.uint8) for _ in range(2))
            self.wt2_f, self.wt2_d = (image(lib.lad_conv_h2_packed_weight_bytes(cin), torch.uint8) for _ in range(2))
        if _s2b3_shape(cin, cout, taps, stride) and base_widths:
            self.wt3_s2f = image(lib.lad_conv_s2b3_packed_weight_bytes(), torch.uint8)
            self.wt3_s2d = image(lib.lad_conv_s2b3_dgrad_packed_weight_bytes(), torch.uint8)


class _BnParams:

    def __init__(self, name, c, views, bufs, dev, conv_bias=None):
        self.name, self.c, self.conv_bias = name, c, conv_bias
        self.g, self.gg = views[name + ".weight"]
        self.b, self.gb = views[name + ".bias"]
        self.rm, self.rv = bufs[name + ".running_mean"], bufs[name + ".running_var"]
        if not (self.rm.is_cuda and self.rm.is_contiguous() and self.rm.dtype == torch.float32):
            raise _hip.LadHipError(f"{name}: running statistics must be contiguous float32 GPU tensors")
        self.fold = (torch.zeros(c, device=dev), torch.zeros(c, device=dev))


class _ConvSpec:

    def __init__(self, name, cin, cout, taps, stride, h_in, w_in, base_widths=True):
        self.name, self.cin, self.cout, self.taps, self.stride = name, cin, cout, taps, stride
        self.h_in, self.w_in = h_in, w_in
        self.h_out = (h_in + stride - 1) // stride
        self.w_out = (w_in + stride - 1) // stride
        self.b3 = _b3_shape(cin, cout, taps, stride) and w_in <= 46 and base_widths
        self.b3_full = self.b3 and cin == 64
        self.b3_wgrad = self.b3 and (cin == 64 or w_in <= 30)
        self.s2b3 = _s2b3_shape(cin, cout, taps, stride) and (w_in + 1) // 2 <= 45 and base_widths
        self.par = None

    def rows(self, B):
        return B * (self.h_in + 1) * (self.w_in + 1) + self.w_in + 2


class _BlockSpec:

    def __init__(self, name):
        self.name = name
        self.conv1 = self.bn1 = self.conv2 = self.bn2 = self.sc_conv = self.sc_bn = None


def block_geometry(stem_cout, filter_sizes, H, W, base_widths):
    blocks = []
    cin, h, w = stem_cout, H, W
    for bi, cout in enumerate(filter_sizes, start=1):
        for j in range(2):
            name = f"block{bi}.{j}"
            stride = 2 if (j == 0 and bi > 1) else 1
            b = _BlockSpec(name)
            b.conv1 = _ConvSpec(name + ".conv1", cin, cout, 9, stride, h, w, base_widths)
            h, w = b.conv1.h_out, b.conv1.w_out
            b.conv2 = _ConvSpec(name + ".conv2", cout, cout, 9, 1, h, w, base_widths)
            if stride != 1 or cin != cout:
                b.sc_conv = _ConvSpec(name + ".shortcut.0", cin, cout, 1, stride, b.conv1.h_in, b.conv1.w_in, base_widths)
            blocks.append(b)
            cin = cout
    return blocks


class _ConvChoice(NamedTuple):
    arith: str
    wgrad: str
    wgrad_bn: bool
    label_fwd: str
    label_dgrad: str


class _BlockChoice(NamedTuple):
    entry: str
    a1_virtual: bool
    bits: bool
    dgrad2_bn: Optional[str]
    dgrad1_bn: Optional[str]
    sc_wgrad_fused: bool
    conv1: _ConvChoice
    conv2: _ConvChoice
    sc: Optional[_ConvChoice]


class _TrainSchedule(NamedTuple):
    blocks: Tuple[_BlockChoice, ...]
    stem_onepass: bool
    images: FrozenSet[Tuple[str, str]]
    opts: Tuple[Tuple[str, object], ...]


_ROW_LIMIT = (1 << 31) - (1 << 20)


def train_schedule(blocks, B, opts, stem_onepass):
    o = dict(opts)

    def arith(cs):
        fits = cs.rows(B) < _ROW_LIMIT if cs.cin == 64 else cs.rows(B) * cs.cin * 4 < _ROW_LIMIT
        if not (o["bf16x3"] and cs.b3 and (cs.cin == 64 or o["bf16x3_32"]) and fits):
            return "f32"
        return "h2" if o["f16x2"] and (cs.cin == 64 or o["f16x2_32"]) else "b3"

    def conv(cs, dgrad_f32=False, label_fwd=None):
        a = arith(cs)
        wg = "f32" if a == "f32" or not cs.b3_wgrad else "h2" if a == "h2" and cs.cin == 64 else "b3c"
        f32_label = f"conv_s{cs.stride}<{cs.cin},{cs.cout},{cs.taps}>"
        return _ConvChoice(a, wg, bool(o["fuse_bn_bwd_wgrad"]) and wg == "h2",
                           label_fwd or (f32_label if a == "f32" else f"conv_{a}<{cs.cin},{cs.cout},{cs.taps}>"),
                           f"conv_s1<{cs.cout},{cs.cin},{cs.taps}>" if a == "f32" or dgrad_f32 else f"conv_{a}<{cs.cout},{cs.cin},{cs.taps}>")

    out = []
    for bi, b in enumerate(blocks):
        c1, c2, sc = b.conv1, b.conv2, b.sc_conv
        a1, a2 = arith(c1), arith(c2)
        below_bits = bi > 0 and out[bi - 1].bits
        entry = "plain"
        if c1.stride != 1 and o["fuse_s2_shortcut"]:
            entry = "s2b3" if o["bf16x3"] and o["s2_b3"] and c1.s2b3 and c1.rows(B) < _ROW_LIMIT else "s2_fused"
        bits = bool(o["relu_bits"]) and sc is None and c1.b3_full and a1 != "f32" and not o["fuse_bn_bwd"]
        dgrad2_bn = "f32" if o["fuse_bn_bwd"] else "split" if o["fuse_bn_bwd_b3"] and a2 != "f32" else None
        if c1.stride != 1:
            fused = entry == "s2b3" or (entry == "s2_fused" and c1.cin == 64 and c1.cout == 32)
            dgrad1_bn = "split" if fused and o["fuse_bn_bwd_b3"] and below_bits else None
        elif bits:
            dgrad1_bn = "split" if o["fuse_bn_bwd_b3"] and below_bits else None
        else:
            dgrad1_bn = "f32" if o["fuse_bn_bwd"] and bi > 0 and blocks[bi - 1].sc_conv is None else None
        s2_label = f"conv_{'s2b3' if entry == 's2b3' else 's2'}<{c1.cin},{c1.cout},9>" if c1.stride != 1 else None
        out.append(_BlockChoice(entry, bool(o["virtual_a1"]) and a2 != "f32" and c2.b3_wgrad, bits, dgrad2_bn, dgrad1_bn,
                                c1.stride != 1 and bool(o["fuse_s2_shortcut_wgrad"]),
                                conv(c1, dgrad1_bn == "f32", s2_label), conv(c2, dgrad2_bn == "f32"), conv(sc) if sc is not None else None))
    images = {(ch.arith if ch.arith == "h2" else "b3c", cs.name) for b, blk in zip(blocks, out)
              for cs, ch in ((b.conv1, blk.conv1), (b.conv2, blk.conv2)) if ch.arith != "f32"}
    images |= {("s2b3", b.conv1.name) for b, blk in zip(blocks, out) if blk.entry == "s2b3"}
    return _TrainSchedule(tuple(out), bool(stem_onepass), frozenset(images), tuple(o.items()))


def conv_s1_entry(arith, cin, in_coef=False, gated=False, bn=None):
    if arith == "h2" and bn != "y":
        return "lad_conv_h2"
    if arith == "b3" and in_coef and not gated and bn is None:
        return "lad_conv_b3c_fwd_f32_bnrelu"
    if arith == "b3" and gated and not in_coef and cin == 64 and bn in (None, "bits"):
        return "lad_conv_b3_dgrad_bnstat" if bn else "lad_conv_b3_fwd_f32_gated"
    if arith == "b3" and not in_coef and not gated and bn in (None, "x"):
        return "lad_conv_b3c_dgrad_bnstat" if bn else "lad_conv_b3c_fwd_f32"
    if arith == "f32" and not in_coef and not gated and bn != "bits":
        return "lad_conv_fwd_bnstat" if bn else "lad_conv_fwd"
    raise _hip.LadHipError(f"no stride-1 convolution kernel for arithmetic {arith!r} at {cin} channels with in_coef={in_coef}, "
                           f"gated={gated}, bn={bn!r}")


def conv_wgrad_entry(kind, in_coef=False, bn=False):
    if kind == "h2":
        return "lad_conv_wgrad_h2_bnbwd" if bn else "lad_conv_wgrad_h2"
    if kind == "b3c" and not bn:
        return "lad_conv_wgrad_b3c"
    if kind == "f32" and not bn and not in_coef:
        return "lad_conv_wgrad"
    raise _hip.LadHipError(f"no weight-gradient kernel for {kind!r} with in_coef={in_coef}, bn={bn}")


def _s2_shortcut_rides(b, opts):
    return bool(opts["f16_s2_shortcut_fused"]) and b.conv1.cin != 32


def _block_fits_lds(b, B, opts, hw=None):
    c = b.conv1
    if b.sc_conv is not None or c.stride != 1 or c.taps != 9 or c.cin != c.cout:
        return False
    h, w = hw if hw is not None else (c.h_in, c.w_in)
    img = (h + 1) * (w + 1)
    if c.cin == 64:
        return bool(opts["strip_block_fused"]) and B >= 256 and img <= 512 and img + w <= 562
    return bool(opts["small_block_fused"]) and c.cin in (16, 32) and B >= 512 and img <= 2048


def _tail_blocks_ok(tail):
    if len(tail) != 4:
        return False
    for k, b in enumerate(tail):
        down = k % 2 == 0
        cin = 32 if k == 0 else 16
        if (b.conv1.cin, b.conv1.cout, b.conv1.taps, b.conv1.stride) != (cin, 16, 9, 2 if down else 1):
            return False
        if (b.conv2.cin, b.conv2.cout, b.conv2.taps, b.conv2.stride) != (16, 16, 9, 1):
            return False
        if down != (b.sc_conv is not None) or (down and (b.sc_conv.cin, b.sc_conv.cout, b.sc_conv.taps, b.sc_conv.stride) != (cin, 16, 1, 2)):
            return False
    return True


class _StreamLayout(NamedTuple):
    B: int
    H: int
    W: int
    half: bool
    mode: str
    run: Optional[Tuple[int, int]]
    n1: int
    band: int
    Ht: Optional[int]
    Hs: Optional[int]
    n_strip: Optional[int]
    n_strip_max: Optional[int]
    img_t_rows: Optional[int]
    stream_row0: Optional[int]
    cat_rows: Optional[int]
    k3: Optional[int]
    H2: Optional[int]
    W2: Optional[int]
    band2: Optional[int]
    Ht2: Optional[int]
    shift2: Optional[int]
    h2s: Optional[int]
    n_strip2: Optional[int]
    n_strip2_max: Optional[int]
    img_t2: Optional[int]
# ... 27 lines not shown
        n1 += 1
    band = 1 + 2 * n1
    if n1 == 0 or H < 4 * band or B < 2:
        return _StreamLayout(B, H, W, bool(half), "per_window", None, n1, band, *(None,) * 20, window_fused, rides, (), (), False, False,
                             (), (), False, False)
    Hs, Ht = B + H - 1, 2 * band
    n_strip = B + H - Ht
    nb = blocks[n1] if n1 < n else None
    direct = bool(half and nb is not None and nb.sc_conv is not None and nb.conv1.stride == 2
                  and (nb.conv1.cin, nb.conv1.cout) == (64, 32) and o["stream_direct"])
    img_t_rows = (Ht + 1) * (W + 1)
    k3 = n1 + 1
    while direct and k3 < n and blocks[k3].conv1.stride == 1 and blocks[k3].sc_conv is None:
        k3 += 1
    n2 = k3 - n1 - 1
    margin2 = 1 + 2 * n2
    band2 = band // 2 + 1 + margin2
    Ht2 = 2 * band2
    shift2 = 2 * (H // 2 - Ht2)
    share2 = bool(direct and o["stream_level2"] and H % 2 == 0 and k3 < n and blocks[k3].sc_conv is not None
                  and blocks[k3].conv1.stride == 2 and (blocks[k3].conv1.cin, blocks[k3].conv1.cout) == (32, 16)
                  and H // 2 >= 2 * Ht2)
    if not (share2 and o["stream_super"]):
        run = None
    mode = "shared2" if share2 else "direct" if direct else "assembled"
    stream_rows = Hs if run is None else run[0] + H - 1
    n_strip_max = n_strip if run is None else run[1] + H - Ht
    stream_row0 = cat_rows = None
    if direct:
        stream_row0 = n_strip_max * img_t_rows
        cat_rows = stream_row0 + (stream_rows + 1) * (W + 1) + W + 2 + (2 * (W + 1) if share2 else 0)
    strip_fused = tuple(bool(half) and _block_fits_lds(b, n_strip, o, (Ht, W)) for b in blocks[:n1])
    stream_fused = tuple(bool(half) and _block_fits_lds(b, 1, o, (stream_rows, W)) for b in blocks[:n1])
    stem_kept = bool(half and o["strip_stem_shared"])
    strip_stem_rows = stem_kept and Ht >= 3 and strip_fused[0] and blocks[0].conv1.cin == 64
    level1 = (n1, band, Ht, Hs, n_strip, n_strip_max, img_t_rows, stream_row0, cat_rows)
    if not share2:
        return _StreamLayout(B, H, W, bool(half), mode, None, *level1, *(None,) * 13, window_fused, rides, stream_fused, strip_fused,
                             stem_kept, strip_stem_rows, (), (), False, False)
    H2, W2 = nb.conv1.h_out, nb.conv1.w_out
    h2s = (stream_rows + 1) // 2
    n_strip2 = B + shift2
    n_strip2_max = n_strip2 if run is None else run[1] + shift2
    img_t2, img_s2 = (Ht2 + 1) * (W2 + 1), (h2s + 1) * (W2 + 1)
    stream2_base = n_strip2_max * img_t2
    rows2 = stream2_base + 2 * img_s2 + W2 + 2
    return _StreamLayout(B, H, W, True, mode, run, *level1, k3, H2, W2, band2, Ht2, shift2, h2s, n_strip2, n_strip2_max, img_t2, img_s2,
                         stream2_base, rows2, window_fused, rides, stream_fused, strip_fused, stem_kept, strip_stem_rows,
                         tuple(_block_fits_lds(b, 2, o, (h2s, W2)) for b in blocks[n1 + 1:k3]),
                         tuple(_block_fits_lds(b, n_strip2, o, (Ht2, W2)) for b in blocks[n1 + 1:k3]),
                         rides[n1] and bool(o["strip2_resident"]) and (nb.conv1.cin, nb.conv1.cout) == (64, 32),
                         bool(o["tail_fused"]) and _tail_blocks_ok(blocks[k3:]))


class _StreamRun:
    __slots__ = ("i0", "S", "B_max", "base", "frames_avail", "cat", "cat2", "stem")

    def __init__(self, i0, S, B_max, base, frames_avail):
        self.i0, self.S, self.B_max = i0, S, B_max
        self.base, self.frames_avail = base, frames_avail
        self.cat = self.cat2 = self.stem = None


class ResNetEngine:
    KERNEL_OPTIONS =("bf16x3", "bf16x3_32", "f16x2", "f16x2_32", "relu_bits", "virtual_a1", "fuse_bn_bwd", "fuse_bn_bwd_b3", "fuse_bn_bwd_wgrad", "fuse_s2_shortcut",
                      "fuse_s2_shortcut_wgrad", "s2_b3")
    INFER_OPTIONS = ("stream_direct", "stream_level2", "stream_super", "strip_block_fused", "small_block_fused", "tail_fused", "strip2_resident",
                     "strip_stem_shared", "f16_s2_shortcut_fused")

    def __init__(self, model):
        self.model = model
        self.device = None
        self._flat_p = self._flat_g = None
        self._plans = {}
        self._step_count = 0
        self._lib = None
        self._grad_dirty = False
        self._train_forwards = 0
        self._weights_version = 0
        self.fuse_bn_bwd = False
        self.overlap_wgrad = False
        self.overlap_wgrad_small = "auto"
        self.stem_onepass = True
        self.bf16x3 = True
        self.fuse_bn_bwd_b3 = True
        self.fuse_bn_bwd_wgrad = True
        self.f16x2 = True
        self.f16x2_32 = True
        self.bf16x3_32 = True
        self.virtual_a1 = True
        self.s2_b3 = True
        self.stream_direct = True
        self.stream_level2 = True
        self.strip_block_fused = True
        self.small_block_fused = True
        self.stream_super = True
        self.tail_fused = True
        self.strip2_resident = True
        self.strip_stem_shared = True
        self._sup_cache = {}
        self._sup_plans = {}
        self._layouts = {}
        self.f16_s2_shortcut_fused = True
        self.fuse_s2_shortcut = True
        self.fuse_s2_shortcut_wgrad = True
        self.defer_wgrad_sums = True
        self._defer_on = False
        self._schedules = {}
        self.relu_bits = True
        self._side = None
        self._side_readers = {}
        self._side_pending = False
        self.debug_capture = None
        self.kernel_events = None
        self.base_widths = list(model.filter_sizes) == list(BASE_WIDTHS)
        if not self.base_widths:
            for k in self.KERNEL_OPTIONS:
                setattr(self, k, False)

    def lib(self):
        if self._lib is None:
            self._lib = _hip.lib()
        return self._lib

    def _named_params(self):
        return list(self.model.named_parameters())

    def ensure_flat(self):
        params = self._named_params()
        dev = params[0][1].device
        if dev.type != "cuda":
            raise _hip.LadHipError("ResNetBigger runs on the MI355X only: call model.set_device('cuda') first "
                                   "(the HIP path has no CPU fallback)")
        ok = self._flat_p is not None and self._flat_p.device == dev
        if ok:
            base = self._flat_p.data_ptr()
            for (name, p), off in zip(params, self._offsets):
                if p.data_ptr() != base + 4 * off or p.dtype != torch.float32:
                    ok = False
                    break
        if ok:
            return
        offs, total = [], 0
        for _, p in params:
            offs.append(total)
            total += _align4(p.numel())
        flat_p = torch.zeros(total, device=dev, dtype=torch.float32)
        flat_g = torch.zeros(total, device=dev, dtype=torch.float32)
        with torch.no_grad():
            for (name, p), off in zip(params, offs):
                view = flat_p[off:off + p.numel()].view(p.shape)
                view.copy_(p.data.to(torch.float32))
                old_grad = p.grad
                p.data = view
                gview = flat_g[off:off + p.numel()].view(p.shape)
                if old_grad is not None:
                    gview.copy_(old_grad)
                    p.grad = gview
        self._flat_p, self._flat_g, self._offsets, self._n_flat = flat_p, flat_g, offs, total
        self._acc_g = None
        self._exp_avg = torch.zeros_like(flat_p)
        self._exp_avg_sq = torch.zeros_like(flat_p)
        self._norm_partials = torch.zeros(int(self.lib().lad_grad_sumsq_partials()), device=dev)
        self._norm_out = torch.zeros(1, device=dev)
        self._step_dev = torch.zeros(1, device=dev, dtype=torch.int64)
        self._rng_counter = torch.zeros(1, device=dev, dtype=torch.int64)
        self._rng_seed = None
        self.device = dev
        self._plans = {}
        self._views = {name: (flat_p[off:off + p.numel()].view(p.shape), flat_g[off:off + p.numel()].view(p.shape))
                       for (name, p), off in zip(params, offs)}
        bns = [m for m in self.model.modules() if isinstance(m, (torch.nn.BatchNorm1d, torch.nn.BatchNorm2d))]
        self._nbt = torch.zeros(len(bns), device=dev, dtype=torch.int64)
        with torch.no_grad():
            for i, m in enumerate(bns):
                self._nbt[i] = m.num_batches_tracked.to(dev)
                m._buffers["num_batches_tracked"] = self._nbt[i]
        self._build_specs()
        self._weights_version += 1
        self._param_list = [p for _, p in params]

    def bump_num_batches_tracked(self):
        self.ensure_flat()
        self._nbt.add_(1)

    def grad_views(self):
        return {k: v[1] for k, v in self._views.items()}

    def attach_grads(self):
        for name, p in self._named_params():
            g = self._views[name][1]
            if p.grad is None or p.grad.data_ptr() != g.data_ptr():
                p.grad = g

    def _build_specs(self):
        m = self.model
        bufs = dict(m.named_buffers())
        lib, dev = self.lib(), self.device

        def bn(name, c, conv_bias=None):
            return _BnParams(name, c, self._views, bufs, dev, conv_bias)

        self.stem_w, self.stem_gw = self._views["conv1.weight"]
        self.stem_cout = self.stem_w.shape[0]
        self.stem_bn = bn("bn1", self.stem_cout)
        self._convs, self._bns = {}, {}
        for b in block_geometry(self.stem_cout, m.filter_sizes, 1, 1, self.base_widths):
            for cs, bn_name in ((b.conv1, ".bn1"), (b.conv2, ".bn2"), (b.sc_conv, ".shortcut.1")):
                if cs is not None:
                    par = self._convs[cs.name] = _ConvParams(cs.name, cs.cin, cs.cout, cs.taps, cs.stride, self.base_widths, self._views, lib, dev)
                    self._bns[b.name + bn_name] = bn(b.name + bn_name, cs.cout, par.b)
            if b.sc_conv is not None:
                self._convs[b.conv1.name].shortcut = self._convs[b.sc_conv.name]
        self._geom_specs = {}
        self._packed = None
        self._folded = None
        self._f16_packed = None
        self._pack_tables = {}
        self._tail_ptrs = None
        self.head_bn2 = bn("bn2", m.linear_layer_size)
        self.head_bn3 = bn("bn3", 32)
        names = ["bn2.weight", "bn2.bias", None, None, "linear1.weight", "linear1.bias", "bn3.weight", "bn3.bias",
                 None, None, "linear2.weight", "linear2.bias"]
        ptrs = []
        for i, n in enumerate(names):
            if n is not None:
                ptrs.append(self._views[n][0].data_ptr())
            else:
                t = {2: self.head_bn2.rm, 3: self.head_bn2.rv, 8: self.head_bn3.rm, 9: self.head_bn3.rv}[i]
                ptrs.append(t.data_ptr())
        self._head_params = (_VP * 12)(*ptrs)
        gnames = ["bn2.weight", "bn2.bias", "linear1.weight", "linear1.bias", "bn3.weight", "bn3.bias",
                  "linear2.weight", "linear2.bias"]
        self._head_grads = (_VP * 8)(*[self._views[n][1].data_ptr() for n in gnames])

    def _blocks_for(self, H, W, partial=False):
        key = (H, W, partial)
        if key in self._geom_specs:
            return self._geom_specs[key]
        blocks = block_geometry(self.stem_cout, self.model.filter_sizes, H, W, self.base_widths)
        for b in blocks:
            b.bn1, b.bn2 = self._bns[b.name + ".bn1"], self._bns[b.name + ".bn2"]
            b.conv1.par, b.conv2.par = self._convs[b.conv1.name], self._convs[b.conv2.name]
            if b.sc_conv is not None:
                b.sc_conv.par, b.sc_bn = self._convs[b.sc_conv.name], self._bns[b.name + ".shortcut.1"]
        h, w = blocks[-1].conv2.h_out, blocks[-1].conv2.w_out
        if partial:
            self._geom_specs[key] = (blocks, h, w, 0)
            return self._geom_specs[key]
        if h < 4 or w < 4:
            raise ValueError(f"input ({H},{W}) is too small: AvgPool2d(4) sees a {h}x{w} map")
        feat = blocks[-1].conv2.cout * (h // 4) * (w // 4)
        if feat != self.model.linear_layer_size:
            raise RuntimeError(f"running_mean should contain {feat} elements not {self.model.linear_layer_size}")
        self._geom_specs[key] = (blocks, h, w, feat)
        return self._geom_specs[key]

    def _plan(self, B, H, W, train):
        key = (B, H, W, train)
        p = self._plans.get(key)
        if p is not None:
            return p
        dev = self.device
        blocks, h4, w4, feat = self._blocks_for(H, W)
        lib = self.lib()

        def act(h, w, c):
            return torch.zeros(int(lib.lad_act_rows(B, h, w)) * c, device=dev, dtype=torch.float32)

        p = {"blocks": blocks, "h4": h4, "w4": w4, "feat": feat}
        c0 = self.stem_cout
        p["stem_a"] = act(H, W, c0)
        p["stem_coef"] = torch.zeros(6 * c0, device=dev)
        if train:
            p["stem_mom"] = torch.zeros(int(lib.lad_stem_moments_doubles()), device=dev, dtype=torch.float64)
            p["stem_mom_ws"] = torch.zeros(int(lib.lad_stem_moments_workspace_doubles()), device=dev, dtype=torch.float64)
            p["stem_bwd_ws"] = torch.zeros(int(lib.lad_stem_bwd_onepass_workspace_floats()), device=dev)
        max_tiles = int(lib.lad_conv_num_tiles(B, H, W))
        for b in blocks:
            if b.conv1.s2b3:
                max_tiles = max(max_tiles, int(lib.lad_conv_s2b3_dgrad_partials(B, b.conv1.h_in, b.conv1.w_in)))
        cmax = max([64] + [b.conv1.cout for b in blocks])
        p["partials"] = torch.zeros(max_tiles * 2 * cmax, device=dev)
        p["partials_sc"] = torch.zeros(max(int(lib.lad_conv_num_tiles(B, b.conv1.h_out, b.conv1.w_out)) * 2 * b.conv1.cout
                                           for b in blocks if b.sc_conv is not None) if any(b.sc_conv is not None for b in blocks) else 0,
                                       device=dev)
        acts = []
        for b in blocks:
            ho, wo, co = b.conv1.h_out, b.conv1.w_out, b.conv1.cout
            d = {"c1": act(ho, wo, co), "a1": act(ho, wo, co), "c2": act(ho, wo, co), "y": act(ho, wo, co),
                 "coef1": torch.zeros(6 * co, device=dev), "coef2": torch.zeros(6 * co, device=dev)}
            if b.sc_conv is not None:
                d["cs"] = act(ho, wo, co)
                d["coefs"] = torch.zeros(6 * co, device=dev)
            elif train and b.conv1.b3_full:
                d["ybits"] = torch.zeros(int(lib.lad_act_rows(B, ho, wo)), device=dev, dtype=torch.int64)
            acts.append(d)
        p["acts"] = acts
        p["pooled"] = torch.zeros(B * feat, device=dev)
        p["probs"] = torch.zeros(B, device=dev)
        if train:
            p["h"] = torch.zeros(B * 32, device=dev)
            p["hstats"] = torch.zeros(2 * feat + 64, device=dev)
            p["metrics"] = torch.zeros(8, device=dev)
            p["head_ws"] = torch.zeros(int(lib.lad_head_workspace_floats(B, feat)), device=dev)
            p["dpooled"] = torch.zeros(B * feat, device=dev)
            levels = {}
            for b, d in zip(blocks, acts):
                ho, wo, co = b.conv1.h_out, b.conv1.w_out, b.conv1.cout
                d["dc1"], d["dc2"] = act(ho, wo, co), act(ho, wo, co)
                if b.conv1.stride != 1:
                    d["aux"] = act(ho, wo, co)
            sizes = {(H, W): c0}
            for b in blocks:
                sizes[(b.conv1.h_out, b.conv1.w_out)] = max(sizes.get((b.conv1.h_out, b.conv1.w_out), 0), b.conv1.cout)
                sizes[(b.conv1.h_in, b.conv1.w_in)] = max(sizes.get((b.conv1.h_in, b.conv1.w_in), 0), b.conv1.cin,
                                                            b.conv1.cout)
            for (h, w), c in sizes.items():
                levels[(h, w)] = [act(h, w, c) for _ in range(4)]
            p["g"] = levels
            ws = max(max(int(lib.lad_conv_wgrad_workspace_floats(cs.cin, cs.cout, cs.taps)),
                         int(lib.lad_conv_s2_wgrad_fused_workspace_floats(cs.cin, cs.cout)) if cs.stride != 1 else 0)
                     for b in blocks for cs in (b.conv1, b.conv2, b.sc_conv) if cs is not None)
            ws = max(ws, int(lib.lad_stem_wgrad_workspace_floats()), int(lib.lad_conv_wgrad_b3c_workspace_floats(32)))
            p["wgrad_ws"] = torch.zeros(ws, device=dev)
            p["wgrad_ws_of"] = {}
            for b in blocks:
                for cs in (b.conv1, b.conv2, b.sc_conv):
                    if cs is not None:
                        n = int(lib.lad_conv_wgrad_workspace_floats(cs.cin, cs.cout, cs.taps))
                        if cs.b3_wgrad:
                            n = max(n, int(lib.lad_conv_wgrad_b3c_workspace_floats(cs.cin)))
                        if cs.stride != 1:
                            n = int(lib.lad_conv_s2_wgrad_fused_workspace_floats(cs.cin, cs.cout)) if cs.taps == 9 else \
                                int(lib.lad_conv_s2_wgrad_workspace_floats(cs.cin, cs.cout, cs.taps))
                        p["wgrad_ws_of"][cs.name] = torch.zeros(n, device=dev)
            p["bn_ws"] = torch.zeros(int(lib.lad_bn_bwd_workspace_floats(cmax)), device=dev)
            p["bcoef"] = torch.zeros(8 * cmax, device=dev)
        self._plans[key] = p
        return p

    def _st(self):
        return _hip.stream_handle(self.device)

    def notify_weights_changed(self):
        self._weights_version += 1

    def _weights_stamp(self):
        return (self._weights_version, sum(p._version for p in self._param_list))

    def _state_tag(self):
        bufs = sum(b._version for b in self.model.buffers())
        return self._weights_stamp() + (bufs, self._train_forwards)

    def _pack_weights(self, need_dgrad, sched=None):
        ver = self._weights_stamp()
        want = sched.images if sched is not None else frozenset()
        have = self._packed
        fresh = have is not None and have[0] == ver
        if fresh and have[1] >= need_dgrad and want <= have[2]:
            return
        lib, st = self.lib(), self._st()
        if not (fresh and have[1] >= need_dgrad):
            table = self._pack_tables.get(need_dgrad)
            if table is None:
                recs = [struct.pack("<QQiiii", par.w.data_ptr(), (par.wt_f if mode == 0 else par.wt_d).data_ptr(), par.cout, par.cin, par.taps, mode)
                        for par in self._convs.values() for mode in ((0, 1) if need_dgrad else (0,))]
                table = self._pack_tables[need_dgrad] = (torch.frombuffer(bytearray(b"".join(recs)), dtype=torch.uint8).to(self.device), len(recs))
            _hip.check(lib.lad_conv_pack_weights_multi(_hip.ptr(table[0]), table[1], st), "lad_conv_pack_weights_multi")
        h2 = []
        for kind, name in sorted(want - have[2] if fresh else want):
            par = self._convs[name]
            if kind == "s2b3":
                _hip.check(lib.lad_conv_s2b3_pack_weights_pair(_hip.ptr(par.w), _hip.ptr(par.shortcut.w), _hip.ptr(par.wt3_s2f),
                                                               _hip.ptr(par.wt3_s2d), st), "lad_conv_s2b3_pack_weights_pair")
            elif kind == "b3c":
                for mode, wt in ((0, par.wt3_f), (1, par.wt3_d)):
                    _hip.check(lib.lad_conv_b3c_pack_weights(_hip.ptr(par.w), mode, _hip.ptr(wt), par.cin, st), "lad_conv_b3c_pack_weights")
            else:
                h2.append(par)
        if h2:
            hkey = ("h2",) + tuple(par.name for par in h2)
            htab = self._pack_tables.get(hkey)
            if htab is None:
                recs = [struct.pack("<QQii", par.w.data_ptr(), wt.data_ptr(), mode, par.cin) for par in h2
                        for mode, wt in ((0, par.wt2_f), (1, par.wt2_d))]
                htab = self._pack_tables[hkey] = (torch.frombuffer(bytearray(b"".join(recs)), dtype=torch.uint8).to(self.device), len(recs))
            _hip.check(lib.lad_conv_h2_pack_weights_multi(_hip.ptr(htab[0]), htab[1], 0, st), "lad_conv_h2_pack_weights_multi")
        self._packed = (ver, need_dgrad or have[1], want | have[2]) if fresh else (ver, need_dgrad, want)

    def _eval_prepare(self, half):
        if not half:
            self._pack_weights(need_dgrad=False)
        tag = self._state_tag()
        lib, st = self.lib(), self._st()
        if self._folded != tag:
            for bn in (self.stem_bn, *self._bns.values()):
                _hip.check(lib.lad_bn_fold(_hip.ptr(bn.g), _hip.ptr(bn.b), _hip.ptr(bn.rm), _hip.ptr(bn.rv), _hip.ptr(bn.conv_bias),
                                           bn.c, _hip.ptr(bn.fold[0]), _hip.ptr(bn.fold[1]), st), "lad_bn_fold " + bn.name)
            self._folded = tag
        if half and self._f16_packed != tag:
            for par in self._convs.values():
                _hip.check(lib.lad_f16_pack_weights(_hip.ptr(par.w), par.cout, par.cin, par.taps, _hip.ptr(par.wt_h), st),
                           "lad_f16_pack_weights " + par.name)
            self._f16_packed = tag

    def _mark(self, label):
        if self.kernel_events is None or label not in self.kernel_events:
            return None
        ev = torch.cuda.Event(enable_timing=True)
        ev.record(torch.cuda.current_stream(self.device))
        return ev

    def _mark_end(self, label, start):
        if start is not None:
            ev = torch.cuda.Event(enable_timing=True)
            ev.record(torch.cuda.current_stream(self.device))
            self.kernel_events[label].append((start, ev))

    def _schedule(self, B, H, W):
        key = (B, H, W, self.stem_onepass) + tuple(getattr(self, k) for k in self.KERNEL_OPTIONS)
        sched = self._schedules.get(key)
        if sched is None:
            sched = self._schedules[key] = train_schedule(self._blocks_for(H, W)[0], B, {k: getattr(self, k) for k in self.KERNEL_OPTIONS},
                                                          self.stem_onepass)
        return sched

    def _conv_s1(self, cs, arith, direction, x, out, B, label=None, *, in_coef=None, bias=None, addend=None, abits=None, partials=None, bn=None):
        bx, bmask, bcoef = bn if bn is not None else (None, None, None)
        fn = conv_s1_entry(arith, cs.cin, in_coef is not None, abits is not None,
                           None if bn is None else "x" if bmask is None else "bits" if bmask.dtype == torch.int64 else "y")
        P, fwd, h, w = _hip.ptr, direction == "fwd", cs.h_in, cs.w_in
        wt = P(getattr(cs.par, {"h2": "wt2_", "b3": "wt3_", "f32": "wt_"}[arith] + ("f" if fwd else "d")))
        cio = (cs.cin, cs.cout) if fwd else (cs.cout, cs.cin)
        if fn == "lad_conv_h2":
            args = (P(x), P(in_coef), wt, P(bias), P(addend), P(abits), P(out), P(partials), P(bx), P(bmask), P(bcoef), B, h, w, cs.cin)
        elif fn == "lad_conv_b3c_fwd_f32":
            args = (P(x), wt, P(bias), P(addend), P(out), P(partials), B, h, w, cs.cin)
        elif fn == "lad_conv_b3c_fwd_f32_bnrelu":
            args = (P(x), P(in_coef), wt, P(bias), P(out), P(partials), B, h, w, cs.cin)
        elif fn == "lad_conv_b3c_dgrad_bnstat":
            args = (P(x), wt, P(addend), P(out), P(partials), P(bx), P(bcoef), B, h, w, cs.cin)
        elif fn == "lad_conv_b3_fwd_f32_gated":
            args = (P(x), wt, P(bias), P(addend), P(abits), P(out), P(partials), B, h, w)
        elif fn == "lad_conv_b3_dgrad_bnstat":
            args = (P(x), wt, P(addend), P(abits), P(out), P(partials), P(bx), P(bmask), P(bcoef), B, h, w)
        elif fn == "lad_conv_fwd":
            args = (P(x), wt, P(bias), P(addend), P(out), P(partials), B, h, w, *cio, cs.taps)
        else:
            args = (P(x), wt, P(addend), P(out), P(partials), P(bx), P(bmask), P(bcoef), B, h, w, *cio, cs.taps)
        t0 = self._mark(label)
        _hip.check(getattr(self.lib(), fn)(*args, self._st()), f"{fn}({direction}) {cs.name}")
        self._mark_end(label, t0)

    def _conv_fwd(self, cs, ch, x, out, partials, B, in_coef=None):
        if cs.stride == 1:
            self._conv_s1(cs, ch.arith, "fwd", x, out, B, ch.label_fwd, in_coef=in_coef, bias=cs.par.b, partials=partials)
            return
        t0 = self._mark(ch.label_fwd)
        _hip.check(self.lib().lad_conv_s2_fwd(_hip.ptr(x), _hip.ptr(cs.par.wt_f), _hip.ptr(cs.par.b), _hip.ptr(out), _hip.ptr(partials),
                                              B, cs.h_in, cs.w_in, cs.cin, cs.cout, cs.taps, self._st()), "lad_conv_s2_fwd " + cs.name)
        self._mark_end(ch.label_fwd, t0)

    def _bn_coef(self, bn, coef, partials, B, h, w):
        lib, st = self.lib(), self._st()
        n_tiles = int(lib.lad_conv_num_tiles(B, h, w))
        _hip.check(lib.lad_bn_finalize(_hip.ptr(partials), n_tiles, bn.c, B * h * w, _hip.ptr(bn.g), _hip.ptr(bn.b),
                                       _hip.ptr(bn.rm), _hip.ptr(bn.rv), 0.1, _hip.ptr(coef), st),
                   "lad_bn_finalize " + bn.name)

    def _bn_coef_pair(self, bn_a, coef_a, part_a, bn_b, coef_b, part_b, B, h, w):
        lib, st = self.lib(), self._st()
        n_tiles = int(lib.lad_conv_num_tiles(B, h, w))
        _hip.check(lib.lad_bn_finalize_pair(_hip.ptr(part_a), _hip.ptr(part_b), n_tiles, bn_a.c, B * h * w,
                                            _hip.ptr(bn_a.g), _hip.ptr(bn_a.b), _hip.ptr(bn_a.rm), _hip.ptr(bn_a.rv), _hip.ptr(coef_a),
                                            _hip.ptr(bn_b.g), _hip.ptr(bn_b.b), _hip.ptr(bn_b.rm), _hip.ptr(bn_b.rv), _hip.ptr(coef_b),
                                            0.1, st), "lad_bn_finalize_pair " + bn_a.name)

    def _bn_act(self, x, coef, res, rcoef, y, B, h, w, c, relu=1):
        _hip.check(self.lib().lad_bn_act(_hip.ptr(x), _hip.ptr(coef), _hip.ptr(res), _hip.ptr(rcoef), _hip.ptr(y), B, h, w, c,
                                         relu, self._st()), "lad_bn_act")

    def forward(self, x, train, labels=None, drop_masks=None):
        self.ensure_flat()
        _hip.require_cuda(x, "x", torch.float32)
        if x.dim() == 4:
            if x.shape[1] != 1:
                raise ValueError("ResNetBigger expects a single input channel: (B,1,T,F)")
            B, _, H, W = x.shape
        elif x.dim() == 3:
            B, H, W = x.shape
        else:
            raise ValueError("x must be (B,1,T,F) or (B,T,F)")
        if B == 0:
            return torch.zeros(0, device=x.device)
        if not train:
            return self._forward_eval(x.view(-1), B, H, W, frame_stride=H, frames_avail=B * H)
        if B < 2:
            raise ValueError("Expected more than 1 value per channel when training, got input size "
                             f"torch.Size([{B}, {self.model.linear_layer_size}])")
        lib, st = self.lib(), self._st()
        p = self._plan(B, H, W, True)
        blocks = p["blocks"]
        sched = p["schedule"] = self._schedule(B, H, W)
        self._pack_weights(need_dgrad=True, sched=sched)
        part = p["partials"]
        if sched.stem_onepass:
            bn = self.stem_bn
# ... 515 lines not shown
        if self._side is None or self._side.device != self.device:
            self._side = torch.cuda.Stream(self.device)
        return self._side

    def _on_side(self, launch, read_buffer, small=False):
        if not (self.overlap_wgrad or (small and self._overlap_small_on())):
            launch(self._st())
            return
        side = self._side_stream()
        side.wait_stream(torch.cuda.current_stream(self.device))
        launch(ctypes.c_void_p(side.cuda_stream))
        ev = torch.cuda.Event()
        ev.record(side)
        self._side_readers[read_buffer.data_ptr()] = ev
        self._side_pending = True

    def _overlap_small_on(self):
        if self.overlap_wgrad_small != "auto":
            return bool(self.overlap_wgrad_small)
        p = getattr(self, "_last_train_plan", None)
        return p is not None and p["saved"][4] >= 256

    def _w(self, buf):
        ev = self._side_readers.pop(buf.data_ptr(), None)
        if ev is not None:
            torch.cuda.current_stream(self.device).wait_event(ev)
        return buf

    def _join_side(self):
        if self._side_pending:
            torch.cuda.current_stream(self.device).wait_stream(self._side)
            self._side_pending = False
            self._side_readers.clear()

    def _wg_ws(self, p, cs):
        return p["wgrad_ws_of"][cs.name] if self._defer_on else p["wgrad_ws"]

    def _conv_wgrad(self, p, cs, kind, x, dout, B, *, in_coef=None, bn=None):
        fn = conv_wgrad_entry(kind, in_coef is not None, bn is not None)
        lib, P, h, w, ws = self.lib(), _hip.ptr, cs.h_in, cs.w_in, self._wg_ws(p, cs)
        if bn is not None:
            dy, bx, bits, coef = bn
            _hip.check(lib.lad_conv_wgrad_h2_bnbwd(P(x), P(in_coef), P(dy), P(bx), P(bits), P(coef), P(p["bcoef"]), P(dout), P(ws), P(cs.par.gw),
                                                   P(cs.par.gb), B, h, w, cs.cin, self._st()), f"{fn} {cs.name}")
        elif kind == "f32":
            self._on_side(lambda st: _hip.check(lib.lad_conv_wgrad(P(x), P(dout), P(ws), P(cs.par.gw), P(cs.par.gb), B, h, w, cs.cin, cs.cout, cs.taps, st),
                                                f"{fn} {cs.name}"), dout, small=cs.cin <= 32)
        else:
            self._on_side(lambda st: _hip.check(getattr(lib, fn)(P(x), P(in_coef), P(dout), P(ws), P(cs.par.gw), P(cs.par.gb), B, h, w, cs.cin, st),
                                                f"{fn} {cs.name}"), dout, small=cs.cin <= 32)

    def backward(self, dprobs=None):
        try:
            self._backward(dprobs)
        except BaseException:
            if self._defer_on:
                self._defer_on = False
                self.lib().lad_wgrad_defer_begin()
                self.lib().lad_wgrad_defer_flush(None)
            raise

    def _backward(self, dprobs):
        p = getattr(self, "_last_train_plan", None)
        if p is None or "saved" not in p:
            raise _hip.LadHipError("backward() without a preceding train-mode forward()")
        x, labels, m1, m2, B, H, W = p["saved"]
        if dprobs is None and labels is None:
            raise _hip.LadHipError("backward() needs dprobs or labels passed to forward()")
        lib, st = self.lib(), self._st()
        blocks, acts, sched = p["blocks"], p["acts"], p["schedule"]
        last = blocks[-1].conv2
        self._defer_on = self.defer_wgrad_sums and not self.overlap_wgrad
        if self._defer_on:
            _hip.check(lib.lad_wgrad_defer_begin(), "lad_wgrad_defer_begin")
        _hip.check(lib.lad_head_bwd(self._head_params, self._head_grads, _hip.ptr(p["pooled"]), _hip.ptr(p["h"]),
                                    _hip.ptr(p["hstats"]), _hip.ptr(p["probs"]), _hip.ptr(dprobs), B, p["feat"], _hip.ptr(m1),
                                    _hip.ptr(m2), _hip.ptr(labels), _hip.ptr(p["head_ws"]), _hip.ptr(p["dpooled"]), st),
                   "lad_head_bwd")
        g_out = p["g"][(last.h_out, last.w_out)]
        dy = g_out[0]
        _hip.check(lib.lad_pool_bwd(_hip.ptr(p["dpooled"]), _hip.ptr(dy), B, p["h4"], p["w4"], last.cout, st), "lad_pool_bwd")
        pre2 = False
        pre2_tiles = 0
        for bi in range(len(blocks) - 1, -1, -1):
            b, a, ch = blocks[bi], acts[bi], sched.blocks[bi]
            c1s, c2s = b.conv1, b.conv2
            ho, wo, co = c1s.h_out, c1s.w_out, c1s.cout
            hi, wi = c1s.h_in, c1s.w_in
            G = p["g"][(ho, wo)]
            free = [t for t in G if t is not dy]
            aux, da1 = (self._w(a["aux"]) if "aux" in a else free[0]), free[1]
            dc2, dc1 = self._w(a["dc2"]), self._w(a["dc1"])
            bits = a["ybits"] if ch.bits else None
            lower = acts[bi - 1]
            fuse2 = ch.bits and ch.conv2.wgrad_bn and not self.overlap_wgrad
            fuse1 = ch.conv1.wgrad_bn and not self.overlap_wgrad
            if ch.bits:
                _hip.check(lib.lad_bn_bwd_bits(_hip.ptr(dy), _hip.ptr(bits), _hip.ptr(a["c2"]), _hip.ptr(a["coef2"]), _hip.ptr(b.bn2.g),
                                               None if fuse2 else _hip.ptr(dc2), _hip.ptr(b.bn2.gg), _hip.ptr(b.bn2.gb), _hip.ptr(p["bn_ws"]),
                                               _hip.ptr(p["bcoef"]), _hip.ptr(p["partials"]) if pre2 else None,
                                               (pre2_tiles or int(lib.lad_conv_num_tiles(B, ho, wo))) if pre2 else 0, B, ho, wo, co, st),
                           "lad_bn_bwd_bits " + b.bn2.name)
            elif b.sc_conv is None:
                self._bn_bwd(p, b.bn2, dy, a["y"], a["c2"], a["coef2"], dc2, B, ho, wo, 1, mode=1, aux=aux, pre=pre2)
            else:
                self._bn_bwd(p, b.bn2, dy, a["y"], a["c2"], a["coef2"], dc2, B, ho, wo, 1, mode=2, aux=aux,
                             sbn=b.sc_bn, xs=a["cs"], scoef=a["coefs"])
            xin, xcoef = (a["c1"], a["coef1"]) if ch.a1_virtual else (a["a1"], None)
            self._conv_wgrad(p, c2s, ch.conv2.wgrad, xin, dc2, B, in_coef=xcoef, bn=(dy, a["c2"], bits, a["coef2"]) if fuse2 else None)
            stat = (a["c1"], None, a["coef1"]) if ch.dgrad2_bn else None
            self._conv_s1(c2s, "f32" if ch.dgrad2_bn == "f32" else ch.conv2.arith, "dgrad", dc2, da1, B, ch.conv2.label_dgrad,
                          bn=stat, partials=p["partials"] if stat else None)
            self._bn_bwd(p, b.bn1, da1, None, a["c1"], a["coef1"], None if fuse1 else dc1, B, ho, wo, 2, mode=0, pre=stat is not None)
            if c1s.stride == 1:
                self._conv_wgrad(p, c1s, ch.conv1.wgrad, a["x"], dc1, B, bn=(da1, a["c1"], None, a["coef1"]) if fuse1 else None)
            if self.debug_capture is not None:
                self.debug_capture[b.name] = {"dy": dy.clone(), "dc2": dc2.clone(), "aux": aux.clone() if bits is None else None, "da1": da1.clone(),
                                              "dc1": dc1.clone()}
            if c1s.stride == 1:
                dx = dy
                if b.sc_conv is not None:
                    self._conv_wgrad(p, b.sc_conv, ch.sc.wgrad, a["x"], aux, B)
                    self._conv_s1(b.sc_conv, ch.sc.arith, "dgrad", aux, da1, B)
                    aux = da1
                stat = (lower["c2"], lower["ybits" if ch.dgrad1_bn == "split" else "y"], lower["coef2"]) if ch.dgrad1_bn else None
                self._conv_s1(c1s, "f32" if ch.dgrad1_bn == "f32" else ch.conv1.arith, "dgrad", dc1, dx, B, ch.conv1.label_dgrad,
                              addend=dy if ch.bits else aux, abits=bits, bn=stat, partials=p["partials"] if stat else None)
                pre2, pre2_tiles = stat is not None, 0
            else:
                dx = p["g"][(hi, wi)][0]
                sc = b.sc_conv

                def s2_wgrad(cs, dout, xin=a["x"]):
                    self._on_side(lambda sst: _hip.check(lib.lad_conv_s2_wgrad(
                        _hip.ptr(xin), _hip.ptr(dout), _hip.ptr(self._wg_ws(p, cs)), _hip.ptr(cs.par.gw), _hip.ptr(cs.par.gb), B, hi, wi, cs.cin, cs.cout,
                        cs.taps, sst), "lad_conv_s2_wgrad " + cs.name), dout, small=cs.cin <= 32)

                if ch.sc_wgrad_fused:
                    self._on_side(lambda sst, c1s=c1s, sc=sc, dc1=dc1, aux=aux, xin=a["x"]: _hip.check(lib.lad_conv_s2_wgrad_fused(
                        _hip.ptr(xin), _hip.ptr(dc1), _hip.ptr(aux), _hip.ptr(self._wg_ws(p, c1s)), _hip.ptr(c1s.par.gw), _hip.ptr(c1s.par.gb),
                        _hip.ptr(sc.par.gw), B, hi, wi, c1s.cin, c1s.cout, sst), "lad_conv_s2_wgrad_fused " + c1s.name), dc1, small=c1s.cin <= 32)
                    if dc1.data_ptr() in self._side_readers:
                        self._side_readers[aux.data_ptr()] = self._side_readers[dc1.data_ptr()]
                else:
                    s2_wgrad(c1s, dc1)
                stat = (lower["c2"], lower["ybits"], lower["coef2"]) if ch.dgrad1_bn else (None, None, None)
                n_part = 0
                if ch.entry == "s2b3":
                    n_part = int(lib.lad_conv_s2b3_dgrad_partials(B, hi, wi))
                    assert not ch.dgrad1_bn or n_part * 2 * 64 <= p["partials"].numel()
                    _hip.check(lib.lad_conv_s2b3_dgrad(_hip.ptr(dc1), _hip.ptr(aux), _hip.ptr(c1s.par.wt3_s2d), _hip.ptr(dx),
                                                       _hip.ptr(p["partials"]) if ch.dgrad1_bn else None, _hip.ptr(stat[0]), _hip.ptr(stat[1]),
                                                       _hip.ptr(stat[2]), B, hi, wi, st), "lad_conv_s2b3_dgrad " + c1s.name)
                elif ch.entry == "s2_fused" and ch.dgrad1_bn:
                    n_part = int(lib.lad_conv_s2_dgrad_partials(B, hi, wi))
                    assert n_part * 2 * 64 <= p["partials"].numel()
                    _hip.check(lib.lad_conv_s2_dgrad_fused_bnstat(_hip.ptr(dc1), _hip.ptr(c1s.par.wt_d), _hip.ptr(aux), _hip.ptr(sc.par.wt_d), _hip.ptr(dx),
                                                                  _hip.ptr(p["partials"]), _hip.ptr(stat[0]), _hip.ptr(stat[1]),
                                                                  _hip.ptr(stat[2]), B, hi, wi, c1s.cin, c1s.cout, st),
                               "lad_conv_s2_dgrad_fused_bnstat " + c1s.name)
                elif ch.entry == "s2_fused":
                    _hip.check(lib.lad_conv_s2_dgrad_fused(_hip.ptr(dc1), _hip.ptr(c1s.par.wt_d), _hip.ptr(aux), _hip.ptr(sc.par.wt_d), _hip.ptr(dx),
                                                           B, hi, wi, c1s.cin, c1s.cout, st), "lad_conv_s2_dgrad_fused " + c1s.name)
                else:
                    _hip.check(lib.lad_conv_s2_dgrad(_hip.ptr(dc1), _hip.ptr(c1s.par.wt_d), _hip.ptr(dx), B, hi, wi, c1s.cin, c1s.cout, 9, 0,
                                                     st), "lad_conv_s2_dgrad " + c1s.name)
                pre2, pre2_tiles = ch.dgrad1_bn is not None, n_part
                if not ch.sc_wgrad_fused:
                    s2_wgrad(sc, aux)
                if ch.entry == "plain":
                    _hip.check(lib.lad_conv_s2_dgrad(_hip.ptr(aux), _hip.ptr(sc.par.wt_d), _hip.ptr(dx), B, hi, wi, sc.cin, sc.cout, 1, 1, st),
                               "lad_conv_s2_dgrad " + sc.name)
            dy = dx
        if sched.stem_onepass:
            bn = self.stem_bn
            _hip.check(lib.lad_stem_bwd_onepass(_hip.ptr(x), _hip.ptr(self.stem_w), _hip.ptr(dy), _hip.ptr(p["stem_coef"]), _hip.ptr(bn.g),
                                                _hip.ptr(p["stem_mom"]), _hip.ptr(p["stem_bwd_ws"]), _hip.ptr(self.stem_gw), _hip.ptr(bn.gg),
                                                _hip.ptr(bn.gb), B, H, W, self.stem_cout, st), "lad_stem_bwd_onepass")
        else:
            groups = int(lib.lad_stem_bn_bwd_groups(B, H, W))
            _hip.check(lib.lad_stem_bn_bwd_sums(_hip.ptr(x), _hip.ptr(self.stem_w), _hip.ptr(dy), _hip.ptr(p["stem_coef"]),
                                                _hip.ptr(p["partials"]), B, H, W, self.stem_cout, st), "lad_stem_bn_bwd_sums")
            bn = self.stem_bn
            _hip.check(lib.lad_bn_bwd(_hip.ptr(dy), None, None, _hip.ptr(p["stem_coef"]), _hip.ptr(bn.g), None, None, None, None,
                                      None, _hip.ptr(bn.gg), _hip.ptr(bn.gb), None, None, _hip.ptr(p["bn_ws"]), _hip.ptr(p["bcoef"]),
                                      _hip.ptr(p["partials"]), groups, B, H, W, bn.c, 2, 0, st), "lad_bn_bwd " + bn.name)
            self._on_side(lambda sst: _hip.check(lib.lad_stem_wgrad_bn(_hip.ptr(x), _hip.ptr(dy), None, _hip.ptr(self.stem_w),
                                                                       _hip.ptr(p["stem_coef"]), _hip.ptr(p["bcoef"]),
                                                                       _hip.ptr(p["wgrad_ws"]), _hip.ptr(self.stem_gw), B, H, W,
                                                                       self.stem_cout, sst), "lad_stem_wgrad_bn"), dy)
        if self._defer_on:
            self._defer_on = False
            self._join_side()
            _hip.check(lib.lad_wgrad_defer_flush(st), "lad_wgrad_defer_flush")
        self._join_side()
        self._grad_dirty = True

    def export_relu_masks(self):
        p = getattr(self, "_last_train_plan", None)
        if p is None or "saved" not in p:
            raise _hip.LadHipError("export_relu_masks() without a preceding train-mode forward()")
        x, labels, m1, m2, B, H, W = p["saved"]

        def unpack(buf, h, w, c):
            body = buf[:B * (h + 1) * (w + 1) * c].view(B, h + 1, w + 1, c)[:, 1:, 1:, :]
            return (body > 0).permute(0, 3, 1, 2).cpu()

        out = {"stem": unpack(p["stem_a"], H, W, self.stem_cout)}
        for b, ch, a in zip(p["blocks"], p["schedule"].blocks, p["acts"]):
            ho, wo, co = b.conv1.h_out, b.conv1.w_out, b.conv1.cout
            if ch.a1_virtual:
                c = a["c1"][:B * (ho + 1) * (wo + 1) * co].view(B, ho + 1, wo + 1, co)[:, 1:, 1:, :].double()
                sc, sh = a["coef1"][:co].double(), a["coef1"][co:2 * co].double()
                out[b.name + ".a1"] = (c * sc + sh > 0).permute(0, 3, 1, 2).cpu()
            else:
                out[b.name + ".a1"] = unpack(a["a1"], ho, wo, co)
            out[b.name + ".y"] = unpack(a["y"], ho, wo, co)
        h = p["h"].view(B, 32).double()
        mean, var = h.mean(0), h.var(0, unbiased=False)
        u = (h - mean) / torch.sqrt(var + 1e-5) * self.head_bn3.g.double() + self.head_bn3.b.double()
        if m2 is not None:
            u = u * m2.double()
        out["head"] = (u > 0).cpu()
        return out

    def reset_optimizer(self):
        self.ensure_flat()
        self._exp_avg.zero_()
        self._exp_avg_sq.zero_()
        self._step_dev.zero_()
        self._step_count = 0

    def reset_dropout_rng(self):
        self.ensure_flat()
        self._rng_counter.zero_()

    def flat_grad(self):
        self.ensure_flat()
        return self._flat_g

    def flat_param(self):
        self.ensure_flat()
        return self._flat_p

    def accumulated_grad(self):
        self.ensure_flat()
        if getattr(self, "_acc_g", None) is None:
            self._acc_g = torch.zeros_like(self._flat_g)
        return self._acc_g

    def accumulate_grad(self, scale):
        acc = self.accumulated_grad()
        _hip.check(self.lib().lad_grad_accumulate(_hip.ptr(acc), _hip.ptr(self._flat_g), self._n_flat, float(scale), self._st()),
                   "lad_grad_accumulate")
        return acc

    def clip_and_step(self, lr=1e-3, betas=(0.9, 0.999), eps=1e-8, max_norm=1.0, grad_scale=1.0, zero_grad=True, grad=None):
# ... 51 lines not shown
```

Baseline: 49510 segments/s.

## Fuse stem BN/wgrad backward into first block's h2 dgrad epilogue

Adds a stem epilogue variant to the h2 conv kernel. The first block's conv1 data gradient is consumed in registers: it is gated by the residual bits, combined with the recomputed stem conv output and BN mask, and reduced into per-tile stem weight and BN sums. A slab finish kernel then produces the stem dw, dgamma and dbeta. This removes the write and re-read of the full 64-channel stem gradient and the separate one-pass stem backward kernel. In exchange the epilogue gets heavier, uses more LDS, and the kernel drops to fewer waves per SIMD.

Result: no change. 49930 segments/s, median of 6 (+0.8%).

```diff
diff --git a/include/lad_hip.h b/include/lad_hip.h
--- a/include/lad_hip.h
+++ b/include/lad_hip.h
@@ -159,6 +159,11 @@
 int lad_conv_h2(const float *in, const float *in_coef, const void *wt, const float *bias, const float *addend,
                 const uint64_t *addend_bits, float *out, float *partials, const float *bn_x, const uint64_t *bn_bits,
                 const float *bn_coef, int64_t batch, int32_t H, int32_t W, int32_t channels, void *stream);
+int64_t lad_conv_h2_dgrad_stem_workspace_floats(int64_t batch, int32_t H, int32_t W);
+int lad_conv_h2_dgrad_stem(const float *in, const void *wt, const float *addend, const uint64_t *addend_bits, const float *feat,
+                           const float *stem_weight, const float *stem_coef, const float *stem_gamma, const double *moments,
+                           float *workspace, int64_t workspace_floats, float *dw, float *dgamma, float *dbeta, int64_t batch,
+                           int32_t H, int32_t W, void *stream);
 int64_t lad_conv_wgrad_b3c_workspace_floats(int32_t channels);
 int lad_conv_wgrad_b3c(const float *in, const float *in_coef, const float *dout, float *workspace, float *dw, float *dbias,
                        int64_t batch, int32_t H, int32_t W, int32_t channels, void *stream);
diff --git a/laughter-detection-icsi_amd/_hip.py b/laughter-detection-icsi_amd/_hip.py
--- a/laughter-detection-icsi_amd/_hip.py
+++ b/laughter-detection-icsi_amd/_hip.py
@@ -67,6 +67,8 @@
     "lad_conv_h2_pack_weights_multi": (c_int, [c_void_p, c_i32, c_i32, c_void_p]),
     "lad_conv_wgrad_h2": (c_int, [c_void_p] * 6 + [c_i64, c_i32, c_i32, c_i32, c_void_p]),
     "lad_conv_h2": (c_int, [c_void_p] * 11 + [c_i64, c_i32, c_i32, c_i32, c_void_p]),
+    "lad_conv_h2_dgrad_stem_workspace_floats": (c_i64, [c_i64, c_i32, c_i32]),
+    "lad_conv_h2_dgrad_stem": (c_int, [c_void_p] * 10 + [c_i64] + [c_void_p] * 3 + [c_i64, c_i32, c_i32, c_void_p]),
     "lad_conv_wgrad_h2_bnbwd": (c_int, [c_void_p] * 11 + [c_i64, c_i32, c_i32, c_i32, c_void_p]),
     "lad_conv_wgrad_b3c_workspace_floats": (c_i64, [c_i32]),
     "lad_conv_wgrad_b3c": (c_int, [c_void_p] * 6 + [c_i64, c_i32, c_i32, c_i32, c_void_p]),
diff --git a/laughter-detection-icsi_amd/csrc/conv_h2.hip b/laughter-detection-icsi_amd/csrc/conv_h2.hip
--- a/laughter-detection-icsi_amd/csrc/conv_h2.hip
+++ b/laughter-detection-icsi_amd/csrc/conv_h2.hip
@@ -106,15 +106,16 @@
 
 constexpr int NSLOT = 3;
 constexpr int H2_EPI_ANY = -1;
+constexpr int H2_EPI_STEM = 64;
 constexpr int h2_epi(bool bias, int addend, bool partials, bool from_bits) {
     return (bias ? 1 : 0) | (addend << 1) | (partials ? 8 : 0) | (from_bits ? 16 : 0);
 }
 template <int C, int RB, bool STAT, bool INBN, int EPI>
-__global__ __launch_bounds__(THREADS, RB == 1 ? 3 : 2) void conv_h2_kernel(const float *__restrict__ in, const unsigned char *__restrict__ wt,
+__global__ __launch_bounds__(THREADS, RB == 1 && EPI != H2_EPI_STEM ? 3 : 2) void conv_h2_kernel(const float *__restrict__ in, const unsigned char *__restrict__ wt,
                                                              const float *__restrict__ bias, const float *addend,
                                                              const unsigned long long *__restrict__ abits, float *out,
                                                              float *__restrict__ partials, Geom g, B3Stat bst,
-                                                             const float *__restrict__ in_coef) {
+                                                             const float *__restrict__ in_coef, H2Stem stem) {
     using K = H2<C>;
     constexpr int NSTAGE = K::NSTAGE, NCT = K::NCT, PLANE_B = K::PLANE_B, TAP_BYTES = K::TAP_BYTES;
     constexpr int TMW = TM * RB, NRT = 2 * RB;
@@ -131,6 +132,8 @@
     unsigned char *a_s = b_s + NSLOT * TAP_BYTES;
     unsigned char *mask_s = smem_b + main_bytes;
     float *smax = reinterpret_cast<float *>(mask_s + TMW);
+    float2 *feat_s = reinterpret_cast<float2 *>(smax + 4);
+    float *stw_s = reinterpret_cast<float *>(feat_s + ((nrows + 1) & ~1));
     const unsigned per_x = (gridDim.x + 7u) / 8u;
     const unsigned tile_id = (blockIdx.x % 8u) * per_x + blockIdx.x / 8u;
     const int64_t q0 = (int64_t)tile_id * TMW;
@@ -195,6 +198,21 @@
         }
     };
 
+    constexpr int NFEAT = (TMW + 2 * 47 + THREADS - 1) / THREADS, NSTW = (STEM_W_FLOATS + THREADS - 1) / THREADS;
+    float fpre[NFEAT], wpre[NSTW], fmean = 0.f;
+    if constexpr (EPI == H2_EPI_STEM) {
+        fmean = (float)stem.mom[STEM_MOM_MEAN];
+#pragma unroll
+        for (int u = 0; u < NFEAT; ++u) {
+            const int j = u * THREADS + tid;
+            uint32_t b, yp, xp;
+            fpre[u] = 0.f;
+            if (j < nrows && decode_row32((uint32_t)(start + j), g, b, yp, xp))
+                fpre[u] = stem.feat[((int64_t)b * stem.H + (yp - 1u)) * stem.W + (xp - 1u)];
+        }
+#pragma unroll
+        for (int u = 0; u < NSTW; ++u) wpre[u] = u * THREADS + tid < STEM_W_FLOATS ? stem.w[u * THREADS + tid] : 0.f;
+    }
     {
         const __amdgpu_buffer_rsrc_t in_r = stage_rsrc(0);
 #pragma unroll
@@ -210,6 +228,16 @@
     }
     LAD_H2_STAMP(1)
     activate(0);
+    if constexpr (EPI == H2_EPI_STEM) {
+#pragma unroll
+        for (int u = 0; u < NFEAT; ++u)
+            if (u * THREADS + tid < nrows) feat_s[u * THREADS + tid] = make_float2(fpre[u], fpre[u] - fmean);
+#pragma unroll
+        for (int u = 0; u < NSTW; ++u) {
+            const int i = u * THREADS + tid;
+            if (i < STEM_W_FLOATS) stw_s[(i % 9) * 64 + i / 9] = wpre[u];
+        }
+    }
     __syncthreads();
     int ktot = tile_exp() + wexp[0];
     put_all(pow2f(ktot - wexp[0]));
@@ -301,6 +329,12 @@
     }
     __syncthreads();
     LAD_H2_STAMP(11)
+    StemSums ss;
+    StemQuad sq;
+    if constexpr (EPI == H2_EPI_STEM) {
+        static_assert(C == 64 && !STAT && !INBN, "the stem consumes a plain 64-channel data gradient");
+        h2_stem_begin(stem, stw_s, sq, ss);
+    }
 #pragma unroll
     for (int rb = 0; rb < RB; ++rb) {
         const int64_t qs = q0 + rb * TM;
@@ -317,21 +351,24 @@
                     for (int j = 0; j < 4; ++j)
                         my[(rr * 16 + (lane >> 4) * 4 + j) * (C + 4) + c * 16 + m] = __builtin_ldexpf(acc[rb * 2 + rr][c][j], -ktot);
         };
-        if constexpr (EPI == H2_EPI_ANY)
+        if constexpr (EPI == H2_EPI_STEM)
+            h2_stem_rows(store_acc, addend, abits, mask_s + rb * TM, reinterpret_cast<float *>(smem_b), feat_s + rb * TM, g.Wp, qs, g.rows, sq, ss);
+        else if constexpr (EPI == H2_EPI_ANY)
             b3_epilogue<C, STAT>(store_acc, bias, addend, abits, out, partials, mask_s + rb * TM, reinterpret_cast<float *>(smem_b), qs, g.rows, bst);
         else
             h2_epilogue<C, STAT, (EPI & 1) != 0, (EPI >> 1) & 3, (EPI & 8) != 0, (EPI & 16) != 0>(
                 store_acc, bias, addend, abits, out, partials, mask_s + rb * TM, reinterpret_cast<float *>(smem_b), qs, g.rows, bst);
     }
+    if constexpr (EPI == H2_EPI_STEM) h2_stem_slab(ss, reinterpret_cast<float *>(smem_b), stem.slabs + (int64_t)tile_id * STEM_BWD_COLS);
     LAD_H2_STAMP(12)
 }
 
 template <int C, int RB>
-size_t h2_lds_bytes(const Geom &g) {
+size_t h2_lds_bytes(const Geom &g, bool stem = false) {
     using K = H2<C>;
     const int nrows = TM * RB + 2 * (g.Wp + 1);
     const size_t main_bytes = std::max<size_t>(NSLOT * K::TAP_BYTES + (size_t)nrows * ROWB, (size_t)TM * (C + 4) * 4);
-    return main_bytes + TM * RB + 16;
+    return main_bytes + TM * RB + 16 + (stem ? stem_lds_floats(nrows) * 4 : 0);
 }
 
 int h2_two_rounds() {
@@ -354,6 +391,7 @@
     B3Stat bst;
     Geom g;
     hipStream_t stream;
+    H2Stem stem;
 };
 
 template <int C, int RB, bool STAT, bool INBN, int EPI>
@@ -364,8 +402,9 @@
         attr_set = true;
     }
     const int64_t tiles = ceil_div(a.g.rows, TM * RB);
-    hipLaunchKernelGGL((conv_h2_kernel<C, RB, STAT, INBN, EPI>), dim3((unsigned)(ceil_div(tiles, 8) * 8)), dim3(THREADS), (h2_lds_bytes<C, RB>(a.g)),
-                       a.stream, a.in, a.wt, a.bias, a.addend, a.abits, a.out, a.partials, a.g, a.bst, a.in_coef);
+    hipLaunchKernelGGL((conv_h2_kernel<C, RB, STAT, INBN, EPI>), dim3((unsigned)(ceil_div(tiles, 8) * 8)), dim3(THREADS),
+                       (h2_lds_bytes<C, RB>(a.g, EPI == H2_EPI_STEM)), a.stream, a.in, a.wt, a.bias, a.addend, a.abits, a.out, a.partials, a.g, a.bst,
+                       a.in_coef, a.stem);
     return check_launch("conv_h2_kernel");
 }
 
@@ -397,7 +436,7 @@
     const Geom g = make_geom(batch, H, W);
     LAD_REQUIRE(g.rows < ((int64_t)1 << 31) && g.img < (1 << 20), "%s: more than 2^31 rows, or an image of more than 2^20 positions", who);
     LAD_REQUIRE(W <= 46, "%s: image too wide for the tile (W = %d)", who, W);
-    const H2Args a{in, in_coef, (const unsigned char *)wt, bias, addend, (const unsigned long long *)abits, out, partials, bst, g, (hipStream_t)stream};
+    const H2Args a{in, in_coef, (const unsigned char *)wt, bias, addend, (const unsigned long long *)abits, out, partials, bst, g, (hipStream_t)stream, H2Stem{}};
     if (ceil_div(g.rows, TM * 2) < h2_two_rounds()) return launch_h2_rb<C, 1, STAT, INBN>(a);
     return launch_h2_rb<C, 2, STAT, INBN>(a);
 }
@@ -448,6 +487,39 @@
     return fail(LAD_ERR_INVALID, "%s: 64 or 32 channels (got %d)", who, channels);
 }
 
+static bool stem_dgrad_rb2(const lad::Geom &g) { return lad::ceil_div(g.rows, lad::b3t::TM * 2) >= h2_two_rounds(); }
+static int64_t stem_dgrad_tiles(const lad::Geom &g) { return lad::ceil_div(g.rows, stem_dgrad_rb2(g) ? lad::b3t::TM * 2 : lad::b3t::TM); }
+extern "C" int64_t lad_conv_h2_dgrad_stem_workspace_floats(int64_t batch, int32_t H, int32_t W) {
+    if (batch < 1 || H < 1 || W < 1) return -1;
+    return (stem_dgrad_tiles(lad::make_geom(batch, H, W)) + 1 + 2 * lad::STEM_FIN_SLICES) * lad::STEM_BWD_COLS;
+}
+
+extern "C" int lad_conv_h2_dgrad_stem(const float *in, const void *wt, const float *addend, const uint64_t *addend_bits, const float *feat,
+                                      const float *stem_weight, const float *stem_coef, const float *stem_gamma, const double *moments,
+                                      float *workspace, int64_t workspace_floats, float *dw, float *dgamma, float *dbeta, int64_t batch,
+                                      int32_t H, int32_t W, void *stream) {
+    using namespace lad;
+    using namespace lad::b3t;
+    const char *who = "lad_conv_h2_dgrad_stem";
+    LAD_REQUIRE(batch >= 1 && H >= 1 && W >= 1, "%s: bad geometry", who);
+    LAD_REQUIRE(in && wt && addend && addend_bits && feat && stem_weight && stem_coef && stem_gamma && moments && workspace && dw && dgamma && dbeta,
+                "%s: null buffer", who);
+    const Geom g = make_geom(batch, H, W);
+    LAD_REQUIRE(g.rows < ((int64_t)1 << 31) && g.img < (1 << 20), "%s: more than 2^31 rows, or an image of more than 2^20 positions", who);
+    LAD_REQUIRE(W <= 46, "%s: image too wide for the tile (W = %d)", who, W);
+    const int64_t tiles = stem_dgrad_tiles(g);
+    const int64_t need = (tiles + 1 + 2 * STEM_FIN_SLICES) * STEM_BWD_COLS;
+    LAD_REQUIRE(workspace_floats >= need, "%s: workspace of %lld floats, %lld needed", who, (long long)workspace_floats, (long long)need);
+    LAD_REQUIRE(((uintptr_t)workspace & 7) == 0, "%s: workspace not 8-byte aligned", who);
+    float *sums = workspace + tiles * STEM_BWD_COLS;
+    double *psum = reinterpret_cast<double *>(workspace + (tiles + 1) * STEM_BWD_COLS);
+    const H2Args a{in, nullptr, (const unsigned char *)wt, nullptr, addend, (const unsigned long long *)addend_bits, nullptr, nullptr,
+                   B3Stat{nullptr, nullptr, nullptr}, g, (hipStream_t)stream, H2Stem{feat, stem_weight, stem_coef, moments, workspace, H, W}};
+    const int rc = stem_dgrad_rb2(g) ? launch_h2_form<64, 2, false, false, H2_EPI_STEM>(a) : launch_h2_form<64, 1, false, false, H2_EPI_STEM>(a);
+    if (rc) return rc;
+    return stem_bwd_finish_slabs(workspace, (int)tiles, sums, psum, moments, stem_weight, stem_coef, stem_gamma, dw, dgamma, dbeta, (hipStream_t)stream);
+}
+
 #ifdef LAD_STAMP
 extern "C" int lad_debug_read_h2_stamps(unsigned long long *host_dst, int64_t n) {
     return hipMemcpyFromSymbol(host_dst, HIP_SYMBOL(lad_dbg_h2), n * sizeof(unsigned long long)) == hipSuccess ? 0 : -2;
diff --git a/laughter-detection-icsi_amd/csrc/lad_b3_tile.h b/laughter-detection-icsi_amd/csrc/lad_b3_tile.h
--- a/laughter-detection-icsi_amd/csrc/lad_b3_tile.h
+++ b/laughter-detection-icsi_amd/csrc/lad_b3_tile.h
@@ -1,6 +1,8 @@
 #pragma once
 #include "lad_common.h"
 #include "lad_device.h"
+#include "lad_bn_math.h"
+#include "lad_stem_taps.h"
 
 namespace lad {
 namespace b3t {
@@ -253,6 +255,134 @@
     }
 }
 
+struct H2Stem {
+    const float *feat;
+    const float *w;
+    const float *coef;
+    const double *mom;
+    float *slabs;
+    int H, W;
+};
+constexpr int STEM_W_FLOATS = 9 * 64;
+__host__ __device__ constexpr int stem_lds_floats(int nrows) { return 2 * ((nrows + 1) & ~1) + STEM_W_FLOATS; }
+
+struct StemSums {
+    float acc[4][9];
+    f32x4 a0, a1;
+};
+struct StemQuad {
+    f32x4 wq[9];
+    float4 fsc, fsh;
+    Norm4 nm;
+};
+__device__ __forceinline__ void h2_stem_begin(const H2Stem &sp, const float *w_s, StemQuad &k, StemSums &ss) {
+    const int c4 = (int)threadIdx.x & 15;
+#pragma unroll
+    for (int tp = 0; tp < 9; ++tp) k.wq[tp] = *reinterpret_cast<const f32x4 *>(w_s + tp * 64 + c4 * 4);
+    k.fsc = *reinterpret_cast<const float4 *>(sp.coef + c4 * 4);
+    k.fsh = *reinterpret_cast<const float4 *>(sp.coef + 64 + c4 * 4);
+    k.nm = load_norm(sp.coef, 64, c4 * 4);
+#pragma unroll
+    for (int c = 0; c < 4; ++c)
+#pragma unroll
+        for (int tp = 0; tp < 9; ++tp) ss.acc[c][tp] = 0.f;
+    ss.a0 = ss.a1 = f32x4{0.f, 0.f, 0.f, 0.f};
+}
+template <class StoreAcc>
+__device__ __forceinline__ void h2_stem_rows(StoreAcc store_acc, const float *addend, const unsigned long long *__restrict__ abits,
+                                             const unsigned char *mask_tile, float *out_s, const float2 *feat_c, int Wp, int64_t q0, int64_t rows,
+                                             const StemQuad &k, StemSums &ss) {
+    constexpr int C = 64, LDO = C + 4, LPR = C / 4, RPI = 64 / LPR, ITER = 32 / RPI, STEP = RPI * C * 4;
+    const int tid = (int)threadIdx.x, lane = tid & 63, wave = tid >> 6;
+    float *my = out_s + wave * 32 * LDO;
+    store_acc(my);
+    const int c4 = lane % LPR, rsub = lane / LPR;
+    const int64_t tile_rows = rows - q0;
+    const int64_t tile_bytes = tile_rows * (C * 4);
+    const int voff = ((wave * 32 + rsub) * C + c4 * 4) * 4;
+    const int woff = (wave * 32 + rsub) * 8;
+    auto gate = [&](u32x4 v, u32x2 w) {
+        const unsigned lo = w.x >> c4, hi = w.y >> c4;
+        v.x = (lo & 1u) ? v.x : 0u;
+        v.y = (lo & 0x10000u) ? v.y : 0u;
+        v.z = (hi & 1u) ? v.z : 0u;
+        v.w = (hi & 0x10000u) ? v.w : 0u;
+        return v;
+    };
+    constexpr int NI = ITER / 2;
+    const float2 *tap_row[3];
+#pragma unroll
+    for (int ky = 0; ky < 3; ++ky) tap_row[ky] = feat_c + wave * 32 + rsub + ky * Wp;
+    const __amdgpu_buffer_rsrc_t add_r = make_rsrc(addend + q0 * C, tile_bytes);
+    const __amdgpu_buffer_rsrc_t bits_r = make_rsrc(abits + q0, tile_rows * 8);
+#pragma unroll
+    for (int i0 = 0; i0 < ITER; i0 += NI) {
+        u32x4 adv[NI];
+        u32x2 wv[NI];
+#pragma unroll
+        for (int u = 0; u < NI; ++u) adv[u] = buf_load16(add_r, voff + (i0 + u) * STEP);
+#pragma unroll
+        for (int u = 0; u < NI; ++u) wv[u] = buf_load8(bits_r, woff + (i0 + u) * RPI * 8);
+#pragma unroll
+        for (int u = 0; u < NI; ++u) {
+            const int row = wave * 32 + (i0 + u) * RPI + rsub;
+            if (mask_tile[row] == 0) continue;
+            f32x4 t = *reinterpret_cast<const f32x4 *>(out_s + row * LDO + c4 * 4);
+            t += __builtin_bit_cast(f32x4, gate(adv[u], wv[u]));
+            float v[9], gt[9];
+#pragma unroll
+            for (int tp = 0; tp < 9; ++tp) {
+                const float2 fc = tap_row[tp / 3][(i0 + u) * RPI + tp % 3];
+                v[tp] = fc.x;
+                gt[tp] = fc.y;
+            }
+            float xa[4] = {0, 0, 0, 0};
+#pragma unroll
+            for (int tp = 0; tp < 9; ++tp)
+#pragma unroll
+                for (int c = 0; c < 4; ++c) xa[c] = fmaf(v[tp], k.wq[tp][c], xa[c]);
+            const float4 xv = make_float4(xa[0], xa[1], xa[2], xa[3]);
+            const float4 d = mask_from_x(make_float4(t.x, t.y, t.z, t.w), xv, k.fsc, k.fsh);
+            const float4 xh = xhat4(xv, k.nm);
+            ss.a0.x += d.x; ss.a0.y += d.y; ss.a0.z += d.z; ss.a0.w += d.w;
+            ss.a1.x = fmaf(d.x, xh.x, ss.a1.x); ss.a1.y = fmaf(d.y, xh.y, ss.a1.y); ss.a1.z = fmaf(d.z, xh.z, ss.a1.z); ss.a1.w = fmaf(d.w, xh.w, ss.a1.w);
+            const float dd[4] = {d.x, d.y, d.z, d.w};
+#pragma unroll
+            for (int tp = 0; tp < 9; ++tp)
+#pragma unroll
+                for (int c = 0; c < 4; ++c) ss.acc[c][tp] = fmaf(gt[tp], dd[c], ss.acc[c][tp]);
+        }
+    }
+}
+__device__ __forceinline__ void h2_stem_slab(StemSums &ss, float *out_s, float *__restrict__ slab) {
+    const int tid = (int)threadIdx.x, lane = tid & 63, wave = tid >> 6, c4 = lane & 15;
+    auto quad = [&](float x) {
+        x += __shfl_xor(x, 16);
+        return x + __shfl_xor(x, 32);
+    };
+#pragma unroll
+    for (int c = 0; c < 4; ++c) {
+#pragma unroll
+        for (int tp = 0; tp < 9; ++tp) ss.acc[c][tp] = quad(ss.acc[c][tp]);
+        ss.a0[c] = quad(ss.a0[c]);
+        ss.a1[c] = quad(ss.a1[c]);
+    }
+    __syncthreads();
+    float *red = out_s + wave * STEM_BWD_COLS;
+    if (lane < 16) {
+#pragma unroll
+        for (int c = 0; c < 4; ++c) {
+#pragma unroll
+            for (int tp = 0; tp < 9; ++tp) red[(c4 * 4 + c) * 9 + tp] = ss.acc[c][tp];
+            red[64 * 9 + c4 * 4 + c] = ss.a0[c];
+            red[64 * 10 + c4 * 4 + c] = ss.a1[c];
+        }
+    }
+    __syncthreads();
+    for (int e = tid; e < STEM_BWD_COLS; e += THREADS)
+        slab[e] = ((out_s[e] + out_s[STEM_BWD_COLS + e]) + out_s[2 * STEM_BWD_COLS + e]) + out_s[3 * STEM_BWD_COLS + e];
+}
+
 template <int TAP_BYTES>
 __device__ __forceinline__ int dma_per_tap(int wave) {
     int n = 0;
diff --git a/laughter-detection-icsi_amd/csrc/lad_common.h b/laughter-detection-icsi_amd/csrc/lad_common.h
--- a/laughter-detection-icsi_amd/csrc/lad_common.h
+++ b/laughter-detection-icsi_amd/csrc/lad_common.h
@@ -58,6 +58,9 @@
 };
 int reduce_slabs(const SlabReduce &d, hipStream_t st);
 
+int stem_bwd_finish_slabs(const float *slabs, int groups, float *sums, double *psum, const double *moments, const float *weight,
+                          const float *coef, const float *gamma, float *dw, float *dgamma, float *dbeta, hipStream_t st);
+
 unsigned int *launch_ticket();
 
 }
diff --git a/laughter-detection-icsi_amd/csrc/lad_device.h b/laughter-detection-icsi_amd/csrc/lad_device.h
--- a/laughter-detection-icsi_amd/csrc/lad_device.h
+++ b/laughter-detection-icsi_amd/csrc/lad_device.h
@@ -43,6 +43,19 @@
     rr = rr >= img ? rr - img : rr;
     const uint32_t yp = __umulhi(rr, g.wp_magic);
     const uint32_t xp = rr - yp * (uint32_t)g.Wp;
+    return ((int64_t)q < g.body) & (yp >= 1u) & (xp >= 1u);
+}
+
+__device__ __forceinline__ bool decode_row32(uint32_t q, const Geom &g, uint32_t &b, uint32_t &yp, uint32_t &xp) {
+    const uint32_t img = (uint32_t)g.img;
+    b = (uint32_t)((double)q * g.inv_img);
+    uint32_t rr = q - b * img;
+    if (rr >= img) {
+        rr -= img;
+        b += 1u;
+    }
+    yp = __umulhi(rr, g.wp_magic);
+    xp = rr - yp * (uint32_t)g.Wp;
     return ((int64_t)q < g.body) & (yp >= 1u) & (xp >= 1u);
 }
 
diff --git a/laughter-detection-icsi_amd/csrc/lad_stem_taps.h b/laughter-detection-icsi_amd/csrc/lad_stem_taps.h
--- a/laughter-detection-icsi_amd/csrc/lad_stem_taps.h
+++ b/laughter-detection-icsi_amd/csrc/lad_stem_taps.h
@@ -45,5 +45,8 @@
     return c.y != 0.0f;
 }
 
+constexpr int STEM_BWD_COLS = 64 * 9 + 2 * 64;
+constexpr int STEM_MOM_MEAN = 54;
+constexpr int STEM_FIN_SLICES = 24;
 
 }
diff --git a/laughter-detection-icsi_amd/csrc/stem.hip b/laughter-detection-icsi_amd/csrc/stem.hip
--- a/laughter-detection-icsi_amd/csrc/stem.hip
+++ b/laughter-detection-icsi_amd/csrc/stem.hip
@@ -488,6 +488,27 @@
         for (int p = 0; p < RL; ++p) sacc += red[p][e];
         slabs[(int64_t)blockIdx.x * BWD1_COLS + e] = sacc;
     }
+}
+static_assert(BWD1_COLS == lad::STEM_BWD_COLS && MOM_N == lad::STEM_MOM_MEAN, "the slab layout conv_h2.hip's stem epilogue writes");
+__device__ __forceinline__ void stem_bwd_tail(int e, const float *tot, const double *__restrict__ mom, const float *__restrict__ w,
+                                              const float *__restrict__ coef, const float *__restrict__ gamma, float *__restrict__ dw,
+                                              float *__restrict__ dgamma, float *__restrict__ dbeta) {
+    if (e >= COUT * 9) {
+        const int c = (e - COUT * 9) & (COUT - 1);
+        if (e < COUT * 10) dbeta[c] = tot[e];
+        else dgamma[c] = tot[e];
+        return;
+    }
+    const int c = e / 9, t = e - c * 9;
+    const double cnt = mom[MOM_N + 1], m = mom[MOM_N];
+    const double mean = (double)coef[2 * COUT + c] + (double)coef[4 * COUT + c], invstd = (double)coef[3 * COUT + c] + (double)coef[5 * COUT + c];
+    const double k1 = (double)gamma[c] * invstd, k2 = (double)tot[COUT * 9 + c] / cnt, k3 = (double)tot[COUT * 10 + c] / cnt;
+    const double g1 = mom[t] - m * cnt;
+    double sgx = 0.0;
+#pragma unroll
+    for (int u = 0; u < 9; ++u) sgx = fma((double)w[c * 9 + u], mom[mom_idx(t, u)] - m * mom[u], sgx);
+    const double gx = invstd * (sgx - mean * g1);
+    dw[e] = (float)(k1 * ((double)tot[e] - k2 * g1 - k3 * gx));
 }
 __global__ __launch_bounds__(64 * CS_PARTS) void stem_bwd_finish_kernel(const float *__restrict__ slabs, float *sums, int groups,
                                                                         const double *__restrict__ mom, const float *__restrict__ w,
@@ -529,24 +550,82 @@
     if (e < n) tot[e] = __hip_atomic_load(sums + e, __ATOMIC_RELAXED, __HIP_MEMORY_SCOPE_AGENT);
     __syncthreads();
     if (e >= n) return;
-    if (e >= COUT * 9) {
-        const int c = (e - COUT * 9) & (COUT - 1);
-        if (e < COUT * 10) dbeta[c] = tot[e];
-        else dgamma[c] = tot[e];
-        return;
-    }
-    const int c = e / 9, t = e - c * 9;
-    const double cnt = mom[MOM_N + 1], m = mom[MOM_N];
-    const double mean = (double)coef[2 * COUT + c] + (double)coef[4 * COUT + c], invstd = (double)coef[3 * COUT + c] + (double)coef[5 * COUT + c];
-    const double k1 = (double)gamma[c] * invstd, k2 = (double)tot[COUT * 9 + c] / cnt, k3 = (double)tot[COUT * 10 + c] / cnt;
-    const double g1 = mom[t] - m * cnt;
-    double sgx = 0.0;
-#pragma unroll
-    for (int u = 0; u < 9; ++u) sgx = fma((double)w[c * 9 + u], mom[mom_idx(t, u)] - m * mom[u], sgx);
-    const double gx = invstd * (sgx - mean * g1);
-    dw[e] = (float)(k1 * ((double)tot[e] - k2 * g1 - k3 * gx));
-}
-
+    stem_bwd_tail(e, tot, mom, w, coef, gamma, dw, dgamma, dbeta);
+}
+__global__ __launch_bounds__(64 * CS_PARTS) void stem_bwd_finish2_kernel(const float *__restrict__ slabs, double *psum, int groups, int per_slice,
+                                                                         const double *__restrict__ mom, const float *__restrict__ w,
+                                                                         const float *__restrict__ coef, const float *__restrict__ gamma,
+                                                                         float *__restrict__ dw, float *__restrict__ dgamma,
+                                                                         float *__restrict__ dbeta, unsigned int *ticket) {
+    constexpr int n = BWD1_COLS;
+    const int o = threadIdx.x & 63, part = threadIdx.x >> 6;
+    const int idx = blockIdx.x * 64 + o;
+    const int lo = blockIdx.y * per_slice, hi = min(groups, lo + per_slice);
+    __shared__ double red[CS_PARTS][64];
+    __shared__ float tot[BWD1_COLS];
+    __shared__ int last_s;
+    double s = 0.0;
+    if (idx < n) {
+        const float *src = slabs + idx;
+        int wg = lo + part;
+        for (; wg + 3 * CS_PARTS < hi; wg += 4 * CS_PARTS) {
+            const float a = src[(int64_t)wg * n], b = src[(int64_t)(wg + CS_PARTS) * n], c = src[(int64_t)(wg + 2 * CS_PARTS) * n],
+                        d = src[(int64_t)(wg + 3 * CS_PARTS) * n];
+            s += (double)a; s += (double)b; s += (double)c; s += (double)d;
+        }
+        for (; wg < hi; wg += CS_PARTS) s += (double)src[(int64_t)wg * n];
+    }
+    red[part][o] = s;
+    __syncthreads();
+    if (part == 0 && idx < n) {
+        double t = 0.0;
+#pragma unroll
+        for (int p = 0; p < CS_PARTS; ++p) t += red[p][o];
+        __hip_atomic_store(psum + (int64_t)blockIdx.y * n + idx, t, __ATOMIC_RELAXED, __HIP_MEMORY_SCOPE_AGENT);
+    }
+    asm volatile("s_waitcnt vmcnt(0)" ::: "memory");
+    __syncthreads();
+    if (threadIdx.x == 0) last_s = __hip_atomic_fetch_add(ticket, 1u, __ATOMIC_RELAXED, __HIP_MEMORY_SCOPE_AGENT) == gridDim.x * gridDim.y - 1;
+    __syncthreads();
+    if (!last_s) return;
+    if (threadIdx.x == 0) __hip_atomic_store(ticket, 0u, __ATOMIC_RELAXED, __HIP_MEMORY_SCOPE_AGENT);
+    const int e = threadIdx.x, slices = (int)gridDim.y;
+    if (e < n) {
+        double t = 0.0;
+        int b = 0;
+        for (; b + 8 <= slices; b += 8) {
+            double v[8];
+#pragma unroll
+            for (int u = 0; u < 8; ++u) v[u] = __hip_atomic_load(psum + (int64_t)(b + u) * n + e, __ATOMIC_RELAXED, __HIP_MEMORY_SCOPE_AGENT);
+#pragma unroll
+            for (int u = 0; u < 8; ++u) t += v[u];
+        }
+        for (; b < slices; ++b) t += __hip_atomic_load(psum + (int64_t)b * n + e, __ATOMIC_RELAXED, __HIP_MEMORY_SCOPE_AGENT);
+        tot[e] = (float)t;
+    }
+    __syncthreads();
+    if (e >= n) return;
+    stem_bwd_tail(e, tot, mom, w, coef, gamma, dw, dgamma, dbeta);
+}
+
+}
+
+int lad::stem_bwd_finish_slabs(const float *slabs, int groups, float *sums, double *psum, const double *moments, const float *weight,
+                               const float *coef, const float *gamma, float *dw, float *dgamma, float *dbeta, hipStream_t st) {
+    constexpr int STEM_FIN_TWO_LEVEL = 1024;
+    unsigned int *ticket = launch_ticket();
+    LAD_REQUIRE(ticket, "stem_bwd_finish_slabs: no ticket");
+    const unsigned col_blocks = (unsigned)ceil_div(BWD1_COLS, 64);
+    if (groups < STEM_FIN_TWO_LEVEL) {
+        hipLaunchKernelGGL(stem_bwd_finish_kernel, dim3(col_blocks), dim3(64 * CS_PARTS), 0, st, slabs, sums, groups, moments, weight, coef, gamma,
+                           dw, dgamma, dbeta, ticket);
+        return check_launch("stem_bwd_finish_kernel");
+    }
+    const int per_slice = (int)ceil_div(groups, STEM_FIN_SLICES);
+    const unsigned slices = (unsigned)ceil_div(groups, per_slice);
+    hipLaunchKernelGGL(stem_bwd_finish2_kernel, dim3(col_blocks, slices), dim3(64 * CS_PARTS), 0, st, slabs, psum, groups, per_slice, moments, weight,
+                       coef, gamma, dw, dgamma, dbeta, ticket);
+    return check_launch("stem_bwd_finish2_kernel");
 }
 
 extern "C" int lad_stem_fwd(const float *feat, const float *weight, float *out, float *stat_partials, int64_t batch,
diff --git a/laughter-detection-icsi_amd/engine.py b/laughter-detection-icsi_amd/engine.py
--- a/laughter-detection-icsi_amd/engine.py
+++ b/laughter-detection-icsi_amd/engine.py
@@ -1,5 +1,6 @@
 import ctypes
 import math
+import os
 import struct
 from typing import FrozenSet, NamedTuple, Optional, Tuple
 
@@ -139,12 +140,13 @@
     stem_onepass: bool
     images: FrozenSet[Tuple[str, str]]
     opts: Tuple[Tuple[str, object], ...]
+    stem_fused: bool = False
 
 
 _ROW_LIMIT = (1 << 31) - (1 << 20)
 
 
-def train_schedule(blocks, B, opts, stem_onepass):
+def train_schedule(blocks, B, opts, stem_onepass, fuse_stem_bwd=False):
     o = dict(opts)
 
     def arith(cs):
@@ -185,7 +187,10 @@
     images = {(ch.arith if ch.arith == "h2" else "b3c", cs.name) for b, blk in zip(blocks, out)
               for cs, ch in ((b.conv1, blk.conv1), (b.conv2, blk.conv2)) if ch.arith != "f32"}
     images |= {("s2b3", b.conv1.name) for b, blk in zip(blocks, out) if blk.entry == "s2b3"}
-    return _TrainSchedule(tuple(out), bool(stem_onepass), frozenset(images), tuple(o.items()))
+    first, c1 = out[0], blocks[0].conv1
+    stem_fused = (bool(fuse_stem_bwd) and bool(stem_onepass) and c1.stride == 1 and c1.cin == 64 and first.conv1.arith == "h2" and first.bits
+                  and first.dgrad1_bn is None)
+    return _TrainSchedule(tuple(out), bool(stem_onepass), frozenset(images), tuple(o.items()), stem_fused)
 
 
 def conv_s1_entry(arith, cin, in_coef=False, gated=False, bn=None):
@@ -379,6 +384,7 @@
         self.overlap_wgrad = False
         self.overlap_wgrad_small = "auto"
         self.stem_onepass = True
+        self.fuse_stem_bwd = os.environ.get("LAD_FUSE_STEM_BWD", "1") != "0"
         self.bf16x3 = True
         self.fuse_bn_bwd_b3 = True
         self.fuse_bn_bwd_wgrad = True
@@ -414,6 +420,7 @@
         if not self.base_widths:
             for k in self.KERNEL_OPTIONS:
                 setattr(self, k, False)
+            self.fuse_stem_bwd = False
 
     def lib(self):
         if self._lib is None:
@@ -572,7 +579,8 @@
         if train:
             p["stem_mom"] = torch.zeros(int(lib.lad_stem_moments_doubles()), device=dev, dtype=torch.float64)
             p["stem_mom_ws"] = torch.zeros(int(lib.lad_stem_moments_workspace_doubles()), device=dev, dtype=torch.float64)
-            p["stem_bwd_ws"] = torch.zeros(int(lib.lad_stem_bwd_onepass_workspace_floats()), device=dev)
+            p["stem_bwd_ws"] = torch.zeros(max(int(lib.lad_stem_bwd_onepass_workspace_floats()),
+                                               int(lib.lad_conv_h2_dgrad_stem_workspace_floats(B, H, W))), device=dev)
         max_tiles = int(lib.lad_conv_num_tiles(B, H, W))
         for b in blocks:
             if b.conv1.s2b3:
@@ -716,11 +724,11 @@
             self.kernel_events[label].append((start, ev))
 
     def _schedule(self, B, H, W):
-        key = (B, H, W, self.stem_onepass) + tuple(getattr(self, k) for k in self.KERNEL_OPTIONS)
+        key = (B, H, W, self.stem_onepass, self.fuse_stem_bwd) + tuple(getattr(self, k) for k in self.KERNEL_OPTIONS)
         sched = self._schedules.get(key)
         if sched is None:
             sched = self._schedules[key] = train_schedule(self._blocks_for(H, W)[0], B, {k: getattr(self, k) for k in self.KERNEL_OPTIONS},
-                                                          self.stem_onepass)
+                                                          self.stem_onepass, self.fuse_stem_bwd)
         return sched
 
     def _conv_s1(self, cs, arith, direction, x, out, B, label=None, *, in_coef=None, bias=None, addend=None, abits=None, partials=None, bn=None):
@@ -1402,6 +1410,7 @@
         _hip.check(lib.lad_pool_bwd(_hip.ptr(p["dpooled"]), _hip.ptr(dy), B, p["h4"], p["w4"], last.cout, st), "lad_pool_bwd")
         pre2 = False
         pre2_tiles = 0
+        stem_fused = sched.stem_fused and self.debug_capture is None
         for bi in range(len(blocks) - 1, -1, -1):
             b, a, ch = blocks[bi], acts[bi], sched.blocks[bi]
             c1s, c2s = b.conv1, b.conv2
@@ -1444,8 +1453,18 @@
                     self._conv_s1(b.sc_conv, ch.sc.arith, "dgrad", aux, da1, B)
                     aux = da1
                 stat = (lower["c2"], lower["ybits" if ch.dgrad1_bn == "split" else "y"], lower["coef2"]) if ch.dgrad1_bn else None
-                self._conv_s1(c1s, "f32" if ch.dgrad1_bn == "f32" else ch.conv1.arith, "dgrad", dc1, dx, B, ch.conv1.label_dgrad,
-                              addend=dy if ch.bits else aux, abits=bits, bn=stat, partials=p["partials"] if stat else None)
+                if bi == 0 and stem_fused:
+                    bn = self.stem_bn
+                    ws = p["stem_bwd_ws"]
+                    t0 = self._mark(ch.conv1.label_dgrad)
+                    _hip.check(lib.lad_conv_h2_dgrad_stem(_hip.ptr(dc1), _hip.ptr(c1s.par.wt2_d), _hip.ptr(dy), _hip.ptr(bits), _hip.ptr(x),
+                                                          _hip.ptr(self.stem_w), _hip.ptr(p["stem_coef"]), _hip.ptr(bn.g), _hip.ptr(p["stem_mom"]),
+                                                          _hip.ptr(ws), ws.numel(), _hip.ptr(self.stem_gw), _hip.ptr(bn.gg), _hip.ptr(bn.gb),
+                                                          B, H, W, st), "lad_conv_h2_dgrad_stem " + c1s.name)
+                    self._mark_end(ch.conv1.label_dgrad, t0)
+                else:
+                    self._conv_s1(c1s, "f32" if ch.dgrad1_bn == "f32" else ch.conv1.arith, "dgrad", dc1, dx, B, ch.conv1.label_dgrad,
+                                  addend=dy if ch.bits else aux, abits=bits, bn=stat, partials=p["partials"] if stat else None)
                 pre2, pre2_tiles = stat is not None, 0
             else:
                 dx = p["g"][(hi, wi)][0]
@@ -1492,7 +1511,9 @@
                     _hip.check(lib.lad_conv_s2_dgrad(_hip.ptr(aux), _hip.ptr(sc.par.wt_d), _hip.ptr(dx), B, hi, wi, sc.cin, sc.cout, 1, 1, st),
                                "lad_conv_s2_dgrad " + sc.name)
             dy = dx
-        if sched.stem_onepass:
+        if stem_fused:
+            pass
+        elif sched.stem_onepass:
             bn = self.stem_bn
             _hip.check(lib.lad_stem_bwd_onepass(_hip.ptr(x), _hip.ptr(self.stem_w), _hip.ptr(dy), _hip.ptr(p["stem_coef"]), _hip.ptr(bn.g),
                                                 _hip.ptr(p["stem_mom"]), _hip.ptr(p["stem_bwd_ws"]), _hip.ptr(self.stem_gw), _hip.ptr(bn.gg),
```
